# coganlab/cross_patient_speech_decoding

Hardware: AMD Instinct MI355X
Metric: ECoG trials/sec seq2seq-RNN training (higher is better)
Workload: dtype bf16x3; 1 GPU; configs[3] per-GPU shard: 8-patient MCCA-aligned input (d = 30), enc 2x bi-GRU H=512, dec 1x GRU, T=200 (T'=20), F=100, full-batch step of 2048 trials per GPU (8 patients x 2048 trials over 8 GPUs), dropout 0.3, teacher forcing 0.5, clip 0.5, AdamW; trials_per_gpu=2048, global_batch=2048, parallelism=dp1, collective=none (single process)

## Files before the change

### cross_patient_speech_decoding_amd/csrc/xps_common.h

```cpp
#pragma once
#include <hip/hip_runtime.h>
#include <stdint.h>
#include <stdio.h>
#include "../../include/xps.h"

typedef float f32x4 __attribute__((ext_vector_type(4)));
typedef float f32x16 __attribute__((ext_vector_type(16)));
typedef double f64x4 __attribute__((ext_vector_type(4)));

void xps_set_error(const char* fmt, ...);

#define XPS_CHECK_ARG(cond, msg)                                  \
    do {                                                          \
        if (!(cond)) {                                            \
            xps_set_error("%s: %s", __func__, msg);               \
            return XPS_E_INVALID;                                 \
        }                                                         \
    } while (0)

#define XPS_CHECK_LAUNCH()                                                        \
    do {                                                                          \
        hipError_t e_ = hipGetLastError();                                        \
        if (e_ != hipSuccess) {                                                   \
            xps_set_error("%s: launch failed: %s", __func__, hipGetErrorString(e_)); \
            return XPS_E_HIP;                                                     \
        }                                                                         \
    } while (0)

struct RowMap {
    long long gs, ld;
    int rpg;
    int fmt = 0;
    __host__ __device__ inline long long off(int i) const {
        return (long long)(i / rpg) * gs + (long long)(i % rpg) * ld;
    }
};

static inline RowMap to_rowmap(const xps_rowmap* r) {
    RowMap m;
    m.gs = r->gs;
    m.ld = r->ld;
    m.rpg = r->rpg < 1 ? 1 : r->rpg;
    m.fmt = r->fmt;
    return m;
}

static inline int cdiv(long long a, long long b) { return (int)((a + b - 1) / b); }

__device__ inline float sigmoidf_acc(float x) { return 1.0f / (1.0f + expf(-x)); }

__device__ inline void rng_pair(unsigned long long seed, long long pair, float& u0, float& u1) {
    unsigned long long z = seed + 0x9E3779B97F4A7C15ull * (unsigned long long)(pair + 1);
    z = (z ^ (z >> 30)) * 0xBF58476D1CE4E5B9ull;
    z = (z ^ (z >> 27)) * 0x94D049BB133111EBull;
    z ^= z >> 31;
    u0 = (float)((unsigned)(z >> 40)) * (1.0f / 16777216.0f);
    u1 = (float)((unsigned)(z >> 8) & 0xFFFFFFu) * (1.0f / 16777216.0f);
}
__device__ inline f32x4 split4_pack(const f32x4 v) {
    typedef __bf16 bf16x8_ __attribute__((ext_vector_type(8)));
    bf16x8_ o;
#pragma unroll
    for (int j = 0; j < 4; ++j) {
        const __bf16 h = (__bf16)v[j];
        o[j] = h;
        o[4 + j] = (__bf16)(v[j] - (float)h);
    }
    return __builtin_bit_cast(f32x4, o);
}
__device__ inline f32x4 dropout_keep4(unsigned long long seed, long long q, float p) {
    float u0, u1, u2, u3;
    rng_pair(seed, 2 * q, u0, u1);
    rng_pair(seed, 2 * q + 1, u2, u3);
    return (f32x4){u0 >= p ? 1.f : 0.f, u1 >= p ? 1.f : 0.f, u2 >= p ? 1.f : 0.f, u3 >= p ? 1.f : 0.f};
}

int xps_internal_gemm_mode();
```

### cross_patient_speech_decoding_amd/csrc/xps_gemm.hip

```cpp
#include <stdlib.h>
#include <string.h>
#include <atomic>
#include "xps_common.h"
#include "xps_gemm_tile.h"
#include "xps_gemm_big.h"
#include "xps_gemm_dma.h"
using namespace xps_tile;
#ifndef XPS_GEMM_DEFAULT_MODE
#define XPS_GEMM_DEFAULT_MODE 1
#endif
namespace {

#ifndef XPS_BF_MI1_WAVES
#define XPS_BF_MI1_WAVES XPS_GEMM_WAVES
#endif
template <bool AK, bool BK, int MI, bool EDGE = false, bool BF = false, bool PRE = false>
__global__ __launch_bounds__(256, (BF && MI == 1) ? XPS_BF_MI1_WAVES : XPS_GEMM_WAVES) void gemm_f32_kernel(
    const float* __restrict__ A, RowMap ra, const float* __restrict__ B, RowMap rb,
    const float* __restrict__ A2, const float* __restrict__ B2, int K2,
    float* __restrict__ C, RowMap rc, const float* __restrict__ bias,
    int M, int N, int K, int kchunk, long long slab_stride, int accumulate, int vecA, int vecB) {
    __shared__ __attribute__((aligned(16))) TileMem<BF, MI> mem;
    const int tiles_n = (N + BN - 1) / BN, tiles = tiles_n * ((M + 64 * MI - 1) / (64 * MI));
    const int lid = xcd_remap(blockIdx.x, gridDim.x);
    const int z = lid / tiles, t = lid % tiles;
    const int kbeg = z * kchunk;
    const int kend = min(K, kbeg + kchunk);
    const int m0 = (t / tiles_n) * (64 * MI), n0 = (t % tiles_n) * BN;
    f32x16 acc[MI][2];
    zero_acc<MI>(acc);
    float nocs = 0.f;
    f32x4 nocs4 = {0.f, 0.f, 0.f, 0.f};
    gemm_accumulate_any<AK, BK, MI, EDGE, BF, PRE>(acc, nocs, nocs4, false, A, ra, B, rb, M, N, K, m0, n0, kbeg, kend, vecA, vecB, mem);
    if (A2) gemm_accumulate_any<AK, BK, MI, EDGE, BF, PRE>(acc, nocs, nocs4, false, A2, ra, B2, rb, M, N, K2, m0, n0, 0, K2, vecA, vecB, mem);
    gemm_store<MI>(acc, C + (long long)z * slab_stride, rc, bias, M, N, m0, n0, accumulate);
}

constexpr int SM_MAXM = 16, SM_SLICES = 16, SM_KC = 1024;
template <bool AK, bool BK>
__global__ __launch_bounds__(1024) void gemm_small_kernel(
    const float* __restrict__ A, RowMap ra, const float* __restrict__ B, RowMap rb,
    const float* __restrict__ A2, const float* __restrict__ B2, int K2,
    float* __restrict__ C, RowMap rc, const float* __restrict__ bias, int M, int N, int K, int accumulate, int vecB) {
    __shared__ __attribute__((aligned(16))) float As[SM_MAXM][SM_KC];
    __shared__ float red[SM_SLICES][SM_MAXM][64];
    const int tid = threadIdx.x, l = tid & 63, w = tid >> 6;
    const int n = blockIdx.x * 64 + l;
    float acc[SM_MAXM];
#pragma unroll
    for (int m = 0; m < SM_MAXM; ++m) acc[m] = 0.f;
    for (int pass = 0; pass < 2; ++pass) {
        const float* __restrict__ Ap = pass ? A2 : A;
        const float* __restrict__ Bp = pass ? B2 : B;
        const int Kp = pass ? K2 : K;
        if (!Ap) break;
        const bool plain_b = rb.rpg >= Kp;
        for (int kc = 0; kc < Kp; kc += SM_KC) {
            const int kn = min(SM_KC, Kp - kc);
            __syncthreads();
            for (int e = tid; e < SM_MAXM * kn; e += 1024) {
                const int m = e / kn, k = e - m * kn;
                As[m][k] = m < M ? (AK ? Ap[ra.off(m) + kc + k] : Ap[ra.off(kc + k) + m]) : 0.f;
            }
            __syncthreads();
            const int kq = (((kn + SM_SLICES - 1) / SM_SLICES) + 3) & ~3;
            const int k0 = w * kq, k1 = min(kn, k0 + kq);
            if (n < N) {
                const long long boff = BK ? rb.off(n) + kc : (long long)n;
                int k = k0;
                for (; k + 3 < k1; k += 4) {
                    float b[4];
                    if (BK && vecB) {
                        const f32x4 v = *reinterpret_cast<const f32x4*>(Bp + boff + k);
                        b[0] = v.x; b[1] = v.y; b[2] = v.z; b[3] = v.w;
                    } else {
#pragma unroll
                        for (int j = 0; j < 4; ++j)
                            b[j] = BK ? Bp[boff + k + j]
                                      : Bp[(plain_b ? (long long)(kc + k + j) * rb.ld : rb.off(kc + k + j)) + boff];
                    }
#pragma unroll
                    for (int m = 0; m < SM_MAXM; ++m) {
                        const f32x4 a = *reinterpret_cast<const f32x4*>(&As[m][k]);
                        acc[m] += a.x * b[0]; acc[m] += a.y * b[1]; acc[m] += a.z * b[2]; acc[m] += a.w * b[3];
                    }
                }
                for (; k < k1; ++k) {
                    const float b = BK ? Bp[boff + k] : Bp[(plain_b ? (long long)(kc + k) * rb.ld : rb.off(kc + k)) + boff];
#pragma unroll
                    for (int m = 0; m < SM_MAXM; ++m) acc[m] += As[m][k] * b;
                }
            }
        }
    }
#pragma unroll
    for (int m = 0; m < SM_MAXM; ++m) red[w][m][l] = acc[m];
    __syncthreads();
    if (w < M && n < N) {
        float v = 0.f;
#pragma unroll
        for (int s = 0; s < SM_SLICES; ++s) v += red[s][w][l];
        if (bias) v += bias[n];
        float* c = C + rc.off(w) + n;
        if (accumulate) v += *c;
        *c = v;
    }
}

struct NtMulti {
    const float* B[4];
    const float* bias[4];
    float* C[4];
};
template <int MI, bool EDGE = false, bool BF = false, bool PRE = false>
__global__ __launch_bounds__(256, (BF && MI == 1) ? XPS_BF_MI1_WAVES : XPS_GEMM_WAVES) void gemm_nt_multi_kernel(
    const float* __restrict__ A, RowMap ra, NtMulti pm, RowMap rb, RowMap rc, int M, int N, int K, int nprob,
    int vecA, int vecB) {
    __shared__ __attribute__((aligned(16))) TileMem<BF, MI> mem;
    const int tiles_n = (N + BN - 1) / BN;
    const int lid = xcd_remap(blockIdx.x, gridDim.x);
    const int per_m = nprob * tiles_n, rem = lid % per_m;
    const int z = rem / tiles_n;
    const int m0 = (lid / per_m) * (64 * MI), n0 = (rem % tiles_n) * BN;
    f32x16 acc[MI][2];
    zero_acc<MI>(acc);
    float nocs = 0.f;
    f32x4 nocs4 = {0.f, 0.f, 0.f, 0.f};
    gemm_accumulate_any<true, true, MI, EDGE, BF, PRE>(acc, nocs, nocs4, false, A, ra, pm.B[z], rb, M, N, K, m0, n0, 0, K, vecA, vecB, mem);
    gemm_store<MI>(acc, pm.C[z], rc, pm.bias[z], M, N, m0, n0, 0);
}


template <int KT>
__global__ __launch_bounds__(512, 1) void proj_ws_kernel(const float* __restrict__ A, long long lda, NtMulti pm, long long ldb, long long ldc,
                                                         int M, int N, int K, int nprob, int preA, int preB) {
    constexpr int KP = 16 * KT;
#ifndef XPS_WS_PAD
#define XPS_WS_PAD 4
#endif
    constexpr int LDH = ((KP / 2 + 63) / 64) * 64 + XPS_WS_PAD;
    constexpr int NV = KP / 32;
    extern __shared__ __attribute__((aligned(16))) unsigned char ws_smem[];
    unsigned* lds = reinterpret_cast<unsigned*>(ws_smem);
    const int tid = threadIdx.x, lane = tid & 63, wave = tid >> 6;
    const int NC = nprob * N, S = (NC + 255) / 256;
    const int lid = xcd_remap(blockIdx.x, gridDim.x);
    const int slice = lid % S, rg = lid / S;
    const int nb = (gridDim.x - slice + S - 1) / S;
    const int c0 = slice * 256 + wave * 32;
    const bool active = c0 < NC;
    const int z = active ? c0 / N : 0, n0 = active ? c0 % N : 0;
    const int li = lane & 31, lk = lane >> 5;

    bf16x8 wh[KT], wl[KT];
    {
        const float* wrow = pm.B[z] + (long long)(n0 + li) * ldb;
#pragma unroll
        for (int kk = 0; kk < KT; ++kk) {
            const int k = 16 * kk + 8 * lk;
            f32x4 v0 = {0.f, 0.f, 0.f, 0.f}, v1 = v0;
            if (active && k < K) v0 = *reinterpret_cast<const f32x4*>(wrow + k);
            if (active && k + 4 < K) v1 = *reinterpret_cast<const f32x4*>(wrow + k + 4);
            bf16x4 h0, l0, h1, l1;
            stage_split(v0, preB != 0, h0, l0);
            stage_split(v1, preB != 0, h1, l1);
            wh[kk] = __builtin_shufflevector(h0, h1, 0, 1, 2, 3, 4, 5, 6, 7);
            wl[kk] = __builtin_shufflevector(l0, l1, 0, 1, 2, 3, 4, 5, 6, 7);
        }
    }
    float bv = 0.f;
    if (active && pm.bias[z]) bv = pm.bias[z][n0 + li];

    const int tiles = (M + 63) / 64;
    auto load_tile = [&](int t, f32x4 (&r)[NV]) {
#pragma unroll
        for (int j = 0; j < NV; ++j) {
            const int v = tid + 512 * j, row = t * 64 + v / (KP / 4), k = 4 * (v % (KP / 4));
            r[j] = (row < M && k < K) ? *reinterpret_cast<const f32x4*>(A + (long long)row * lda + k) : f32x4{0.f, 0.f, 0.f, 0.f};
        }
    };
    auto store_tile = [&](const f32x4 (&r)[NV], int buf) {
        unsigned* hi = lds + (size_t)buf * 2 * 64 * LDH;
        unsigned* lo = hi + 64 * LDH;
#pragma unroll
        for (int j = 0; j < NV; ++j) {
            const int v = tid + 512 * j, row = v / (KP / 4), kd = 2 * (v % (KP / 4));
            bf16x4 h, l;
            stage_split(r[j], preA != 0, h, l);
// ... 151 lines not shown
        for (int u = 0; u < 8; ++u) v[u] = p[(long long)(z + 4 * u) * stride];
#pragma unroll
        for (int u = 0; u < 8; ++u) s += v[u];
    }
    for (; z < splits; z += 4) s += p[(long long)z * stride];
    return s;
}

__device__ inline f32x4 slab_sum4(const float* __restrict__ p, long long stride, int splits, int w) {
    f32x4 s = {0.f, 0.f, 0.f, 0.f};
    int z = w;
    for (; z + 28 < splits; z += 32) {
        f32x4 v[8];
#pragma unroll
        for (int u = 0; u < 8; ++u) v[u] = *reinterpret_cast<const f32x4*>(p + (long long)(z + 4 * u) * stride);
#pragma unroll
        for (int u = 0; u < 8; ++u) s += v[u];
    }
    for (; z < splits; z += 4) s += *reinterpret_cast<const f32x4*>(p + (long long)z * stride);
    return s;
}

__global__ __launch_bounds__(256) void gemm_tn_grouped_reduce(TnGroup g, const float* __restrict__ ws) {
    __shared__ f32x4 part[4][RED_OUT];
    const int l = threadIdx.x & 63, w = threadIdx.x >> 6;
    const long long idx = ((long long)blockIdx.x * RED_OUT + l) * 4;
    const bool live = idx < g.total_out;
    int pi = 0;
    long long base = 0;
    if (live) {
#pragma unroll 1
        for (int i = 0; i < g.n; ++i) {
            const long long sz = tn_split_stride((long long)((g.p[i].M + BM - 1) / BM) * g.p[i].tiles_n, g.p[i].M, g.p[i].colsum != nullptr);
            if (idx < base + sz) { pi = i; break; }
            base += sz;
        }
    }
    const TnProb& P = g.p[pi];
    const long long tile_floats = (long long)((P.M + BM - 1) / BM) * P.tiles_n * TN_TILE;
    const long long split_stride = tn_split_stride(tile_floats / TN_TILE, P.M, P.colsum != nullptr);
    const long long e = idx - base;
    part[w][l] = live ? slab_sum4(ws + P.slab_off + e, split_stride, P.splits, w) : f32x4{0.f, 0.f, 0.f, 0.f};
    __syncthreads();
    if (w == 0 && live) {
        const f32x4 s4 = (part[0][l] + part[1][l]) + (part[2][l] + part[3][l]);
#pragma unroll
        for (int c = 0; c < 4; ++c) {
            float* dst = nullptr;
            bool is_cs = false;
            if (e < tile_floats) {
                const int tile = (int)(e / TN_TILE);
                int r, cc;
                slab_decode((int)(e % TN_TILE) + c, r, cc);
                const int row = (tile / P.tiles_n) * BM + r, col = (tile % P.tiles_n) * BN + cc;
                if (row < P.M && col < P.N)
                    dst = P.C + (P.rc.rpg >= P.M ? (long long)row * P.rc.ld : P.rc.off(row)) + col;
            } else {
                is_cs = true;
                if (e - tile_floats + c < P.M) dst = P.colsum + (e - tile_floats + c);
            }
            if (dst) {
                float s = s4[c];
                if ((P.accumulate & 1) || ((P.accumulate & 2) && is_cs)) s += *dst;
                *dst = s;
            }
        }
    }
}

__global__ __launch_bounds__(256) void gemm_tn_grouped_reduce_flat(TnGroup g, const float* __restrict__ ws) {
    const long long idx = ((long long)blockIdx.x * 256 + threadIdx.x) * 4;
    const bool live = idx < g.total_out;
    int pi = 0;
    long long base = 0;
    if (live) {
#pragma unroll 1
        for (int i = 0; i < g.n; ++i) {
            const long long sz = tn_split_stride((long long)((g.p[i].M + BM - 1) / BM) * g.p[i].tiles_n, g.p[i].M, g.p[i].colsum != nullptr);
            if (idx < base + sz) { pi = i; break; }
            base += sz;
        }
    }
    const TnProb& P = g.p[pi];
    const long long tile_floats = (long long)((P.M + BM - 1) / BM) * P.tiles_n * TN_TILE;
    const long long split_stride = tn_split_stride(tile_floats / TN_TILE, P.M, P.colsum != nullptr);
    const long long e = idx - base;
    if (live) {
        f32x4 s4 = {0.f, 0.f, 0.f, 0.f};
        const float* src = ws + P.slab_off + e;
        int z = 0;
        for (; z + 8 <= P.splits; z += 8) {
            f32x4 v[8];
#pragma unroll
            for (int u = 0; u < 8; ++u) v[u] = *reinterpret_cast<const f32x4*>(src + (long long)(z + u) * split_stride);
#pragma unroll
            for (int u = 0; u < 8; ++u) s4 += v[u];
        }
        {
            f32x4 v[8];
#pragma unroll
            for (int u = 0; u < 8; ++u)
                v[u] = z + u < P.splits ? *reinterpret_cast<const f32x4*>(src + (long long)(z + u) * split_stride) : f32x4{0.f, 0.f, 0.f, 0.f};
#pragma unroll
            for (int u = 0; u < 8; ++u) s4 += v[u];
        }
#pragma unroll
        for (int c = 0; c < 4; ++c) {
            float* dst = nullptr;
            bool is_cs = false;
            if (e < tile_floats) {
                const int tile = (int)(e / TN_TILE);
                int r, cc;
                slab_decode((int)(e % TN_TILE) + c, r, cc);
                const int row = (tile / P.tiles_n) * BM + r, col = (tile % P.tiles_n) * BN + cc;
                if (row < P.M && col < P.N)
                    dst = P.C + (P.rc.rpg >= P.M ? (long long)row * P.rc.ld : P.rc.off(row)) + col;
            } else {
                is_cs = true;
                if (e - tile_floats + c < P.M) dst = P.colsum + (e - tile_floats + c);
            }
            if (dst) {
                float s = s4[c];
                if ((P.accumulate & 1) || ((P.accumulate & 2) && is_cs)) s += *dst;
                *dst = s;
            }
        }
    }
}

extern __shared__ __attribute__((aligned(16))) unsigned char big_smem[];

template <bool AK, bool BK, bool DEEP, int FMT = -1>
__device__ inline void big_accumulate(f32x16 (&acc)[4][2], f32x4& csum, bool want_csum, const float* __restrict__ A, long long lda,
                                      const float* __restrict__ B, long long ldb, int m0, int n0, int kbeg, int kend,
                                      const bool preA = false, const bool preB = false) {
    if constexpr (DEEP) {
        xps_big::BigStage32& st = *reinterpret_cast<xps_big::BigStage32*>(big_smem);
        xps_big::BigLoader32<AK> la;
        xps_big::BigLoader32<BK> lb;
        la.init(A, lda, m0, kbeg, threadIdx.x);
        lb.init(B, ldb, n0, kbeg, threadIdx.x);
        xps_big::big_pipeline32<AK, BK>(acc, csum, want_csum, la, lb, (kend - kbeg) / 32, st, preA, preB);
    } else {
        xps_big::BigStage& st = *reinterpret_cast<xps_big::BigStage*>(big_smem);
        xps_big::BigLoader<AK> la;
        xps_big::BigLoader<BK> lb;
        la.init(A, lda, m0, kbeg, threadIdx.x);
        lb.init(B, ldb, n0, kbeg, threadIdx.x);
        if constexpr (FMT >= 0) xps_big::big_pipeline_t<AK, BK, (FMT & 1) != 0, (FMT & 2) != 0>(acc, csum, want_csum, la, lb, (kend - kbeg) / BKT, st);
        else xps_big::big_pipeline<AK, BK>(acc, csum, want_csum, la, lb, (kend - kbeg) / BKT, st, preA, preB);
    }
}

template <bool AK, bool BK, bool DEEP, int FMT = 0>
__global__ __launch_bounds__(512, 1) void gemm_big_kernel(const float* __restrict__ A, long long lda, const float* __restrict__ B,
                                                           long long ldb, const float* __restrict__ A2, const float* __restrict__ B2,
                                                           int K2, float* __restrict__ C, long long ldc,
                                                           const float* __restrict__ bias, int N, int K, int accumulate, int fmt) {
    const int tiles_n = FMT == 5 ? 1 : N / xps_big::TN;
    const int lid = xcd_remap(blockIdx.x, gridDim.x);
    const int m0 = (lid / tiles_n) * xps_big::TM, n0 = (lid % tiles_n) * xps_big::TN;
    f32x16 acc[4][2];
    xps_big::big_zero(acc);
    f32x4 nocs = {0.f, 0.f, 0.f, 0.f};
    if constexpr (FMT == 5) {
        const bool act = (int)((threadIdx.x >> 6) & 3) * 64 < N;
        xps_big::direct_dma_pipeline<!BK>(acc, A, lda, B, ldb, m0, 0, 0, K / 32, big_smem, act);
        if (A2) xps_big::direct_dma_pipeline<!BK>(acc, A2, lda, B2, ldb, m0, 0, 0, K2 / 32, big_smem, act);
        xps_big::big_store_c_masked(acc, C, ldc, bias, m0, N, accumulate);
        return;
    }
    if constexpr (FMT == 4) {
        xps_big::direct_dma_pipeline<!BK>(acc, A, lda, B, ldb, m0, n0, 0, K / 32, big_smem);
        if (A2) xps_big::direct_dma_pipeline<!BK>(acc, A2, lda, B2, ldb, m0, n0, 0, K2 / 32, big_smem);
    } else {
        big_accumulate<AK, BK, DEEP, DEEP ? -1 : FMT>(acc, nocs, false, A, lda, B, ldb, m0, n0, 0, K, !DEEP && (fmt & 1) != 0, !DEEP && (fmt & 2) != 0);
        if (A2) big_accumulate<AK, BK, DEEP, DEEP ? -1 : FMT>(acc, nocs, false, A2, lda, B2, ldb, m0, n0, 0, K2, !DEEP && (fmt & 1) != 0, !DEEP && (fmt & 2) != 0);
    }
    xps_big::big_store_c(acc, C, ldc, bias, m0, n0, accumulate);
}

template <bool DEEP, bool DMA = false>
__global__ __launch_bounds__(512, 1) void gemm_big_nt_multi_kernel(const float* __restrict__ A, long long lda, NtMulti pm, long long ldb,
                                                                    long long ldc, int N, int K, int nprob, int fmt) {
    const int tiles_n = N / xps_big::TN;
    const int lid = xcd_remap(blockIdx.x, gridDim.x);
    const int per_m = nprob * tiles_n, rem = lid % per_m;
    const int z = rem / tiles_n;
    const int m0 = (lid / per_m) * xps_big::TM, n0 = (rem % tiles_n) * xps_big::TN;
    f32x16 acc[4][2];
    xps_big::big_zero(acc);
    f32x4 nocs = {0.f, 0.f, 0.f, 0.f};
    if constexpr (DMA) xps_big::direct_dma_pipeline<false>(acc, A, lda, pm.B[z], ldb, m0, n0, 0, K / 32, big_smem);
    else big_accumulate<true, true, DEEP>(acc, nocs, false, A, lda, pm.B[z], ldb, m0, n0, 0, K, !DEEP && (fmt & 1) != 0, !DEEP && (fmt & 2) != 0);
    xps_big::big_store_c(acc, pm.C[z], ldc, pm.bias[z], m0, n0, 0);
}

template <bool DEEP>
__global__ __launch_bounds__(512, 1) void gemm_big_tn_kernel(TnGroup g, float* __restrict__ ws) {
    const int lid = xcd_remap(blockIdx.x, gridDim.x);
    int pi = -1;
#pragma unroll 1
    for (int i = 0; i < g.n; ++i)
        if (g.p[i].big && lid >= g.p[i].block_start) pi = i;
    const TnProb& P = g.p[pi];
    const int local = lid - P.block_start;
    const int tiles_n = P.N / xps_big::TN, ntiles = (P.M / xps_big::TM) * tiles_n;
    const int tile = local % ntiles, z = local / ntiles;
    const int tm = tile / tiles_n, tn = tile % tiles_n;
    const int kbeg = z * P.kchunk, kend = min(P.K, kbeg + P.kchunk);
    const long long ntiles128 = (long long)(P.M / BM) * P.tiles_n;
    const long long split_stride = tn_split_stride(ntiles128, P.M, P.colsum != nullptr);
    float* slab = ws + P.slab_off + (long long)z * split_stride;
    const bool want_cs = P.colsum && tn == 0;
    f32x16 acc[4][2];
    xps_big::big_zero(acc);
    if (!DEEP && P.big == 2) {
        f32x16 cacc;
#pragma unroll
        for (int r = 0; r < 16; ++r) cacc[r] = 0.f;
        const int per = (8 + tiles_n - 1) / tiles_n;
        const int cs_lo = min(8, tn * per), cs_hi = min(8, cs_lo + per);
        const bool cs_here = P.colsum && cs_lo < cs_hi;
        if (cs_here) xps_big::tn_dma_pipeline<true>(acc, cacc, P.A, P.ra.ld, P.B, P.rb.ld, tm * xps_big::TM, tn * xps_big::TN, kbeg, (kend - kbeg) / BKT, big_smem, cs_lo, cs_hi);
        else xps_big::tn_dma_pipeline<false>(acc, cacc, P.A, P.ra.ld, P.B, P.rb.ld, tm * xps_big::TM, tn * xps_big::TN, kbeg, (kend - kbeg) / BKT, big_smem);
        float* subd[4];
#pragma unroll
        for (int s = 0; s < 4; ++s)
            subd[s] = slab + ((long long)(2 * tm + (s >> 1)) * P.tiles_n + 2 * tn + (s & 1)) * TN_TILE;
        xps_big::big_slab_store(acc, subd);
        if (cs_here) xps_big::dma_colsum_store(cacc, slab + ntiles128 * TN_TILE + tm * xps_big::TM, cs_lo, cs_hi);
        return;
    }
    f32x4 csum = {0.f, 0.f, 0.f, 0.f};
    big_accumulate<false, false, DEEP>(acc, csum, want_cs, P.A, P.ra.ld, P.B, P.rb.ld, tm * xps_big::TM, tn * xps_big::TN, kbeg, kend,
                                       !DEEP && (P.vecA & 2) != 0, !DEEP && (P.vecB & 2) != 0);
    float* sub[4];
#pragma unroll
    for (int s = 0; s < 4; ++s)
        sub[s] = slab + ((long long)(2 * tm + (s >> 1)) * P.tiles_n + 2 * tn + (s & 1)) * TN_TILE;
    xps_big::big_slab_store(acc, sub);
    if (want_cs) {
        float* red = reinterpret_cast<float*>(big_smem);
        const int tid = threadIdx.x;
        *reinterpret_cast<f32x4*>(&red[(tid >> 6) * 256 + (tid & 63) * 4]) = csum;
        __syncthreads();
        if (tid < 256) {
            float v = 0.f;
#pragma unroll
            for (int w = 0; w < 8; ++w) v += red[w * 256 + tid];
            slab[ntiles128 * TN_TILE + tm * xps_big::TM + tid] = v;
        }
    }
}

__global__ __launch_bounds__(256) void splitk_reduce_kernel(const float* __restrict__ slabs, int splits, long long slab_stride,
                                                            float* __restrict__ C, RowMap rc, int M, int N, int accumulate) {
    __shared__ float part[4][RED_OUT];
    const int l = threadIdx.x & 63, w = threadIdx.x >> 6;
    const long long idx = (long long)blockIdx.x * RED_OUT + l;
    const bool live = idx < (long long)M * N;
    part[w][l] = live ? slab_sum(slabs + idx, slab_stride, splits, w) : 0.f;
    __syncthreads();
    if (w == 0 && live) {
        float s = (part[0][l] + part[1][l]) + (part[2][l] + part[3][l]);
        float* p = C + rc.off((int)(idx / N)) + (int)(idx % N);
        if (accumulate) s += *p;
        *p = s;
    }
}

inline bool aligned16(const void* p) { return (reinterpret_cast<uintptr_t>(p) & 15) == 0; }
inline bool map_vec_ok(const float* p, const RowMap& r) {
    return aligned16(p) && (r.ld % 4 == 0) && (r.gs % 4 == 0);
}
inline int split4_flag(const float* p, const RowMap& r, long long extent) {
    if (r.fmt == 0) return 0;
    if (r.fmt != 1 || !map_vec_ok(p, r) || extent % 4 != 0) return -1;
    return 2;
}

int tn_splits(int M, int N, int K) {
    long long tiles = (long long)cdiv(M, BM) * cdiv(N, BN);
    int want = (int)((768 + tiles - 1) / tiles);
    int maxs = cdiv(K, 256);
    int s = want < maxs ? want : maxs;
    if (s < 1) s = 1;
    if (s > 256) s = 256;
    return s;
}

}

namespace {
std::atomic<int>& gemm_mode() {
    static std::atomic<int> mode([] {
        const char* e = getenv("XPS_GEMM_PRECISION");
        if (e && (!strcmp(e, "fp32") || !strcmp(e, "f32") || !strcmp(e, "0"))) return 0;
        if (e && (!strcmp(e, "bf16x3") || !strcmp(e, "1"))) return 1;
        return XPS_GEMM_DEFAULT_MODE;
    }());
    return mode;
}
inline bool bf_mode() { return gemm_mode().load(std::memory_order_relaxed) == 1; }

inline bool use_small_tiles(int M, int N, int K = 0) {
    static const int thr = [] {
        const char* e = getenv("XPS_GEMM_SMALL_TILE_BLOCKS");
        int v = e ? atoi(e) : -1;
        return v >= 0 ? v : 2048;
    }();
    const long long n128 = (long long)cdiv(M, 128) * cdiv(N, BN);
    static const bool longk = [] { const char* e = getenv("XPS_GEMM_LONGK_128"); return !(e && e[0] == '0'); }();
    if (longk && K >= 1024 && n128 >= 512) return false;
    return M > 64 && n128 < thr;
}

std::atomic<int>& big_switch() {
    static std::atomic<int> on([] { const char* e = getenv("XPS_GEMM_BIG"); return (e && e[0] == '0') ? 0 : 1; }());
    return on;
}
inline bool big_enabled() { return big_switch().load(std::memory_order_relaxed) != 0 && bf_mode(); }
inline bool dma_enabled() { const char* e = getenv("XPS_GEMM_DMA"); return !(e && e[0] == '0'); }
inline bool proj_ws_enabled() { const char* e = getenv("XPS_PROJ_WS"); return !(e && e[0] == '0'); }
inline bool big_plain(const float* p, const RowMap& r, int rows) { return aligned16(p) && r.ld % 4 == 0 && r.rpg >= rows; }
constexpr int BIG_LDS = (int)sizeof(xps_big::BigStage), BIG_LDS32 = (int)sizeof(xps_big::BigStage32);
constexpr int BIG_TN_LDS = BIG_LDS > xps_big::DMA_LDS ? BIG_LDS : xps_big::DMA_LDS;
template <typename Kern>
inline bool big_prepare(Kern kern, int bytes) {
    return hipFuncSetAttribute(reinterpret_cast<const void*>(kern), hipFuncAttributeMaxDynamicSharedMemorySize, bytes) == hipSuccess;
}
inline bool big_deep_allowed() {
    static const bool on = [] { const char* e = getenv("XPS_GEMM_BIG_DEEP"); return e && e[0] == '1'; }();
    return on;
}
inline int big_min_tiles() {
    static const int v = [] { const char* e = getenv("XPS_GEMM_BIG_MIN_TILES"); int x = e ? atoi(e) : 0; return x > 0 ? x : 192; }();
    return v;
}

inline int device_cus() {
    static const int cus = [] {
        int dev = 0, n = 0;
        if (hipGetDevice(&dev) == hipSuccess && hipDeviceGetAttribute(&n, hipDeviceAttributeMultiprocessorCount, dev) == hipSuccess && n > 0) return n;
        return 256;
    }();
    return cus;
}
inline int big_split_rows(int M, int tiles_per_row_tile) {
    static const bool on = [] { const char* e = getenv("XPS_GEMM_BIG_TAIL"); return !(e && e[0] == '0'); }();
    const int cus = device_cus();
    const long long mt = M / xps_big::TM, total = mt * tiles_per_row_tile;
    const long long rounds = total / cus, rem = total % cus;
    if (!on || rounds < 1 || rem == 0 || rem * 4 > (long long)cus * 3) return M;
    const long long mb = (rounds * cus) / tiles_per_row_tile;
    if (mb < 1 || mb >= mt) return M;
    return (int)(mb * xps_big::TM);
}

template <bool AK, bool BK>
int launch_gemm(const float* A, const RowMap& ra, const float* B, const RowMap& rb, const float* A2, const float* B2, int K2,
                float* C, const RowMap& rc, const float* bias, int M, int N, int K, int accumulate, hipStream_t st) {
    const int kchunk = ((K + BKT - 1) / BKT) * BKT + BKT;
    int vecA = (int)(map_vec_ok(A, ra) && (!A2 || map_vec_ok(A2, ra)));
    int vecB = (int)(map_vec_ok(B, rb) && (!B2 || map_vec_ok(B2, rb)));
    int fA = split4_flag(A, ra, AK ? K : M), fB = split4_flag(B, rb, BK ? K : N);
    if (A2 && fA > 0) fA = split4_flag(A2, ra, AK ? K2 : M);
    if (B2 && fB > 0) fB = split4_flag(B2, rb, BK ? K2 : N);
    if (fA < 0 || fB < 0 || ((fA | fB) && (!bf_mode() || M <= SM_MAXM))) return -2;
    vecA |= fA; vecB |= fB;
    const int fmt = (fA ? 1 : 0) | (fB ? 2 : 0);
    if (M <= SM_MAXM) {
        hipLaunchKernelGGL((gemm_small_kernel<AK, BK>), dim3(cdiv(N, 64)), dim3(1024), 0, st, A, ra, B, rb, A2, B2, K2, C, rc,
                           bias, M, N, K, accumulate, vecB);
        return hipGetLastError() == hipSuccess ? 0 : -1;
    }
    if constexpr (AK && !BK) {
        if (big_enabled() && dma_enabled() && fmt == 3 && N < xps_big::TN && N % 4 == 0 && rb.ld >= xps_big::TN && M % xps_big::TM == 0 &&
            M / xps_big::TM >= 96 && K % 32 == 0 && K2 % 32 == 0 && K + K2 >= 512 && big_plain(A, ra, M) && big_plain(B, rb, K) &&
            (!A2 || (big_plain(A2, ra, M) && big_plain(B2, rb, K2))) && rc.rpg >= M) {
            constexpr int lds = xps_big::direct_dma_lds<true>();
            static const bool ready5 = big_prepare(gemm_big_kernel<true, false, false, 5>, lds);
            if (ready5) {
                hipLaunchKernelGGL((gemm_big_kernel<true, false, false, 5>), dim3(M / xps_big::TM), dim3(xps_big::NTHR), lds, st,
                                   A, ra.ld, B, rb.ld, A2, B2, K2, C, rc.ld, bias, N, K, accumulate, fmt);
                return hipGetLastError() == hipSuccess ? 0 : -1;
            }
        }
    }
    if (big_enabled() && M % xps_big::TM == 0 && N % xps_big::TN == 0 && K % BKT == 0 && K2 % BKT == 0 && K >= 64 &&
        (long long)(M / xps_big::TM) * (N / xps_big::TN) >= big_min_tiles() &&
        big_plain(A, ra, AK ? M : K) && big_plain(B, rb, BK ? N : K) && (!A2 || (big_plain(A2, ra, AK ? M : K2) && big_plain(B2, rb, BK ? N : K2))) &&
        rc.rpg >= M) {
        static const bool ready = big_prepare(gemm_big_kernel<AK, BK, false, 0>, BIG_LDS) && big_prepare(gemm_big_kernel<AK, BK, false, 1>, BIG_LDS) &&
                                  big_prepare(gemm_big_kernel<AK, BK, false, 2>, BIG_LDS) && big_prepare(gemm_big_kernel<AK, BK, false, 3>, BIG_LDS) &&
                                  big_prepare(gemm_big_kernel<AK, BK, true>, BIG_LDS32);
        if (ready) {
            const int Mfull = M;
            M = big_split_rows(M, N / xps_big::TN);
            const dim3 bgrid((M / xps_big::TM) * (N / xps_big::TN));
            const int Mtail = Mfull - M;
            auto run_tail = [&]() -> int {
                if (Mtail <= 0) return 0;
                const float* At = AK ? A + (long long)M * ra.ld : A + M;
                const float* A2t = A2 ? (AK ? A2 + (long long)M * ra.ld : A2 + M) : nullptr;
                return launch_gemm<AK, BK>(At, ra, B, rb, A2t, B2, K2, C + (long long)M * rc.ld, rc, bias, Mtail, N, K, accumulate, st);
            };
            bool dma_done = false;
            if constexpr (AK) {
                if (fmt == 3 && K % 32 == 0 && K2 % 32 == 0 && dma_enabled()) {
                    constexpr int lds = xps_big::direct_dma_lds<!BK>();
                    static const bool ready4 = big_prepare(gemm_big_kernel<AK, BK, false, 4>, lds);
                    if (ready4) {
                        hipLaunchKernelGGL((gemm_big_kernel<AK, BK, false, 4>), bgrid, dim3(xps_big::NTHR), lds, st,
                                           A, ra.ld, B, rb.ld, A2, B2, K2, C, rc.ld, bias, N, K, accumulate, fmt);
                        dma_done = true;
                    }
                }
            }
            if (dma_done) {
            } else if (big_deep_allowed() && K % 32 == 0 && K2 % 32 == 0 && fmt == 0)
                hipLaunchKernelGGL((gemm_big_kernel<AK, BK, true>), bgrid, dim3(xps_big::NTHR), BIG_LDS32, st,
                                   A, ra.ld, B, rb.ld, A2, B2, K2, C, rc.ld, bias, N, K, accumulate, fmt);
            else if (fmt == 0)
                hipLaunchKernelGGL((gemm_big_kernel<AK, BK, false, 0>), bgrid, dim3(xps_big::NTHR), BIG_LDS, st,
                                   A, ra.ld, B, rb.ld, A2, B2, K2, C, rc.ld, bias, N, K, accumulate, fmt);
            else if (fmt == 1)
                hipLaunchKernelGGL((gemm_big_kernel<AK, BK, false, 1>), bgrid, dim3(xps_big::NTHR), BIG_LDS, st,
                                   A, ra.ld, B, rb.ld, A2, B2, K2, C, rc.ld, bias, N, K, accumulate, fmt);
            else if (fmt == 2)
                hipLaunchKernelGGL((gemm_big_kernel<AK, BK, false, 2>), bgrid, dim3(xps_big::NTHR), BIG_LDS, st,
                                   A, ra.ld, B, rb.ld, A2, B2, K2, C, rc.ld, bias, N, K, accumulate, fmt);
            else
                hipLaunchKernelGGL((gemm_big_kernel<AK, BK, false, 3>), bgrid, dim3(xps_big::NTHR), BIG_LDS, st,
                                   A, ra.ld, B, rb.ld, A2, B2, K2, C, rc.ld, bias, N, K, accumulate, fmt);
            if (hipGetLastError() != hipSuccess) return -1;
            return run_tail();
        }
    }
#define XPS_LAUNCH_GEMM(MI_, EDGE_, BF_)                                                                              \
    do {                                                                                                              \
        if (BF_ && fmt)                                                                                               \
            hipLaunchKernelGGL((gemm_f32_kernel<AK, BK, MI_, EDGE_, BF_, BF_>), grid, dim3(256), 0, st, A, ra, B, rb, A2, B2, K2, C, rc, \
                               bias, M, N, K, kchunk, 0LL, accumulate, vecA, vecB);                                   \
        else                                                                                                          \
            hipLaunchKernelGGL((gemm_f32_kernel<AK, BK, MI_, EDGE_, BF_>), grid, dim3(256), 0, st, A, ra, B, rb, A2, B2, K2, C, rc, \
                               bias, M, N, K, kchunk, 0LL, accumulate, vecA, vecB);                                   \
    } while (0)
    const bool bf = bf_mode();
    if (use_small_tiles(M, N, K + K2)) {
        dim3 grid(cdiv(N, BN) * cdiv(M, 64));
        const bool edge = (M % 64) || (N % BN);
        if (bf) { if (edge) XPS_LAUNCH_GEMM(1, true, true); else XPS_LAUNCH_GEMM(1, false, true); }
        else { if (edge) XPS_LAUNCH_GEMM(1, true, false); else XPS_LAUNCH_GEMM(1, false, false); }
    } else {
        dim3 grid(cdiv(N, BN) * cdiv(M, 128));
        const bool edge = (M % 128) || (N % BN);
        if (bf) { if (edge) XPS_LAUNCH_GEMM(2, true, true); else XPS_LAUNCH_GEMM(2, false, true); }
        else { if (edge) XPS_LAUNCH_GEMM(2, true, false); else XPS_LAUNCH_GEMM(2, false, false); }
    }
#undef XPS_LAUNCH_GEMM
    return hipGetLastError() == hipSuccess ? 0 : -1;
}
}

extern "C" int xps_gemm_nt_f32(const float* A, const xps_rowmap* ra_, const float* B, const xps_rowmap* rb_,
                               float* C, const xps_rowmap* rc_, const float* bias,
                               int M, int N, int K, int accumulate, void* stream) {
    XPS_CHECK_ARG(A && B && C && ra_ && rb_ && rc_, "null argument");
    XPS_CHECK_ARG(M >= 0 && N >= 0 && K >= 0, "negative size");
    if (M == 0 || N == 0) return XPS_OK;
    RowMap ra = to_rowmap(ra_), rb = to_rowmap(rb_), rc = to_rowmap(rc_);
    const int lrc = launch_gemm<true, true>(A, ra, B, rb, nullptr, nullptr, 0, C, rc, bias, M, N, K, accumulate, (hipStream_t)stream);
    if (lrc == -2) {
        xps_set_error("xps_gemm_nt_f32: XPS_FMT_SPLIT4 operand needs bf16x3 mode, M > 16, 16-byte aligned rows and a contiguous extent that is a multiple of 4");
        return XPS_E_INVALID;
    }
    if (lrc) {
        xps_set_error("xps_gemm_nt_f32: launch failed: %s", hipGetErrorString(hipGetLastError()));
        return XPS_E_HIP;
    }
    return XPS_OK;
}

extern "C" int xps_gemm_nn_f32(const float* A, const xps_rowmap* ra_, const float* B, const xps_rowmap* rb_,
                               float* C, const xps_rowmap* rc_,
                               int M, int N, int K, int accumulate, void* stream) {
    XPS_CHECK_ARG(A && B && C && ra_ && rb_ && rc_, "null argument");
    XPS_CHECK_ARG(M >= 0 && N >= 0 && K >= 0, "negative size");
    if (M == 0 || N == 0) return XPS_OK;
    RowMap ra = to_rowmap(ra_), rb = to_rowmap(rb_), rc = to_rowmap(rc_);
    const int lrc = launch_gemm<true, false>(A, ra, B, rb, nullptr, nullptr, 0, C, rc, nullptr, M, N, K, accumulate, (hipStream_t)stream);
    if (lrc == -2) {
        xps_set_error("xps_gemm_nn_f32: XPS_FMT_SPLIT4 operand needs bf16x3 mode, M > 16, 16-byte aligned rows and a contiguous extent that is a multiple of 4");
        return XPS_E_INVALID;
    }
    if (lrc) {
        xps_set_error("xps_gemm_nn_f32: launch failed: %s", hipGetErrorString(hipGetLastError()));
        return XPS_E_HIP;
    }
    return XPS_OK;
}

extern "C" int xps_gemm_nt_multi_f32(const float* A, const xps_rowmap* ra_, const float* const* B, const xps_rowmap* rb_,
                                     float* const* C, const xps_rowmap* rc_, const float* const* bias, int nprob,
                                     int M, int N, int K, void* stream) {
    XPS_CHECK_ARG(A && B && C && ra_ && rb_ && rc_, "null argument");
    XPS_CHECK_ARG(nprob >= 1 && nprob <= 4, "1..4 problems");
    XPS_CHECK_ARG(M >= 0 && N >= 0 && K >= 0, "negative size");
    if (M == 0 || N == 0) return XPS_OK;
    RowMap ra = to_rowmap(ra_), rb = to_rowmap(rb_), rc = to_rowmap(rc_);
    NtMulti pm;
    bool vb = true;
    for (int i = 0; i < 4; ++i) {
        const int j = i < nprob ? i : 0;
        XPS_CHECK_ARG(B[j] && C[j], "null problem pointer");
        pm.B[i] = B[j]; pm.C[i] = C[j]; pm.bias[i] = bias ? bias[j] : nullptr;
        vb = vb && map_vec_ok(B[j], rb);
    }
    int vecA = (int)map_vec_ok(A, ra), vecB = (int)vb;
    int fA = split4_flag(A, ra, K), fB = 0;
    for (int i = 0; i < nprob && fB >= 0; ++i) fB = split4_flag(B[i], rb, K);
    if (fA < 0 || fB < 0 || ((fA | fB) && !bf_mode())) {
        xps_set_error("xps_gemm_nt_multi_f32: XPS_FMT_SPLIT4 operand needs bf16x3 mode, 16-byte aligned rows and K %% 4 == 0");
        return XPS_E_INVALID;
    }
    vecA |= fA; vecB |= fB;
    const int fmt = (fA ? 1 : 0) | (fB ? 2 : 0);
    if (bf_mode() && proj_ws_enabled() && K >= 32 && K <= 256 && K % 4 == 0 && N % 32 == 0 && (long long)nprob * N >= 256 && M >= 4096 &&
        vecA && vb && ra.rpg >= M && rb.rpg >= N && rc.rpg >= M) {
        const int KT = 2 * ((K + 31) / 32);
        static const int cus = [] {
            int dev = 0, n = 0;
            if (hipGetDevice(&dev) == hipSuccess && hipDeviceGetAttribute(&n, hipDeviceAttributeMultiprocessorCount, dev) == hipSuccess && n > 0) return n;
            return 256;
        }();
        const int S = cdiv((long long)nprob * N, 256), tiles = cdiv(M, 64);
        int grid = cus < tiles * S ? cus : tiles * S;
        grid = (grid / S) * S;
        if (grid >= S) {
#define XPS_LAUNCH_WS(KT_)                                                                                                            \
    do {                                                                                                                              \
        static const bool ok_ = big_prepare(proj_ws_kernel<KT_>, proj_ws_lds(KT_));                                                    \
        if (!ok_) { xps_set_error("xps_gemm_nt_multi_f32: cannot reserve %d bytes of LDS", proj_ws_lds(KT_)); return XPS_E_HIP; }       \
        hipLaunchKernelGGL(proj_ws_kernel<KT_>, dim3(grid), dim3(512), proj_ws_lds(KT_), (hipStream_t)stream, A, ra.ld, pm, rb.ld, rc.ld, \
                           M, N, K, nprob, fA ? 1 : 0, fB ? 1 : 0);                                                                      \
    } while (0)
            switch (KT) {
                case 2: XPS_LAUNCH_WS(2); break;
                case 4: XPS_LAUNCH_WS(4); break;
                case 6: XPS_LAUNCH_WS(6); break;
                case 8: XPS_LAUNCH_WS(8); break;
                case 10: XPS_LAUNCH_WS(10); break;
                case 12: XPS_LAUNCH_WS(12); break;
                case 14: XPS_LAUNCH_WS(14); break;
                default: XPS_LAUNCH_WS(16); break;
            }
#undef XPS_LAUNCH_WS
            XPS_CHECK_LAUNCH();
            return XPS_OK;
        }
    }
    if (big_enabled() && M % xps_big::TM == 0 && N % xps_big::TN == 0 && K % BKT == 0 && K >= 64 && vb &&
        (long long)(M / xps_big::TM) * (N / xps_big::TN) * nprob >= big_min_tiles() &&
        big_plain(A, ra, M) && rb.rpg >= N && rc.rpg >= M) {
        static const bool ready = big_prepare(gemm_big_nt_multi_kernel<false>, BIG_LDS) && big_prepare(gemm_big_nt_multi_kernel<true>, BIG_LDS32);
        if (ready) {
            const int Mfull = M;
            M = big_split_rows(M, (N / xps_big::TN) * nprob);
            const dim3 bgrid((M / xps_big::TM) * (N / xps_big::TN) * nprob);
            static const bool ready_dma = big_prepare(gemm_big_nt_multi_kernel<false, true>, xps_big::direct_dma_lds<false>());
            if (fmt == 3 && K % 32 == 0 && dma_enabled() && ready_dma)
                hipLaunchKernelGGL((gemm_big_nt_multi_kernel<false, true>), bgrid, dim3(xps_big::NTHR), xps_big::direct_dma_lds<false>(),
                                   (hipStream_t)stream, A, ra.ld, pm, rb.ld, rc.ld, N, K, nprob, fmt);
            else if (big_deep_allowed() && K % 32 == 0 && fmt == 0)
                hipLaunchKernelGGL(gemm_big_nt_multi_kernel<true>, bgrid, dim3(xps_big::NTHR), BIG_LDS32, (hipStream_t)stream, A, ra.ld, pm,
                                   rb.ld, rc.ld, N, K, nprob, fmt);
            else
                hipLaunchKernelGGL(gemm_big_nt_multi_kernel<false>, bgrid, dim3(xps_big::NTHR), BIG_LDS,
                               (hipStream_t)stream, A, ra.ld, pm, rb.ld, rc.ld, N, K, nprob, fmt);
            XPS_CHECK_LAUNCH();
            if (Mfull > M) {
                float* Ct[4];
                for (int i = 0; i < nprob; ++i) Ct[i] = C[i] + (long long)M * rc.ld;
                return xps_gemm_nt_multi_f32(A + (long long)M * ra.ld, ra_, B, rb_, Ct, rc_, bias, nprob, Mfull - M, N, K, stream);
            }
            return XPS_OK;
        }
    }
#define XPS_LAUNCH_NTM(MI_, EDGE_, BF_)                                                                                  \
    do {                                                                                                                 \
        if (BF_ && fmt)                                                                                                  \
            hipLaunchKernelGGL((gemm_nt_multi_kernel<MI_, EDGE_, BF_, BF_>), dim3(cdiv(N, BN) * cdiv(M, 64 * MI_) * nprob), dim3(256), 0, \
                               (hipStream_t)stream, A, ra, pm, rb, rc, M, N, K, nprob, vecA, vecB);                        \
        else                                                                                                             \
            hipLaunchKernelGGL((gemm_nt_multi_kernel<MI_, EDGE_, BF_>), dim3(cdiv(N, BN) * cdiv(M, 64 * MI_) * nprob), dim3(256), 0,    \
                               (hipStream_t)stream, A, ra, pm, rb, rc, M, N, K, nprob, vecA, vecB);                        \
    } while (0)
    const bool bf = bf_mode();
    if (use_small_tiles(M, N * nprob, K)) {
        const bool edge = (M % 64) || (N % BN);
        if (bf) { if (edge) XPS_LAUNCH_NTM(1, true, true); else XPS_LAUNCH_NTM(1, false, true); }
        else { if (edge) XPS_LAUNCH_NTM(1, true, false); else XPS_LAUNCH_NTM(1, false, false); }
    } else {
        const bool edge = (M % 128) || (N % BN);
        if (bf) { if (edge) XPS_LAUNCH_NTM(2, true, true); else XPS_LAUNCH_NTM(2, false, true); }
        else { if (edge) XPS_LAUNCH_NTM(2, true, false); else XPS_LAUNCH_NTM(2, false, false); }
    }
#undef XPS_LAUNCH_NTM
    XPS_CHECK_LAUNCH();
    return XPS_OK;
}

extern "C" int xps_gemm_nn2_f32(const float* A1, const float* B1, int K1, const float* A2, const float* B2, int K2,
                                const xps_rowmap* ra_, const xps_rowmap* rb_, float* C, const xps_rowmap* rc_,
                                int M, int N, int accumulate, void* stream) {
    XPS_CHECK_ARG(A1 && B1 && A2 && B2 && C && ra_ && rb_ && rc_, "null argument");
    XPS_CHECK_ARG(M >= 0 && N >= 0 && K1 >= 0 && K2 >= 0, "negative size");
    if (M == 0 || N == 0) return XPS_OK;
    RowMap ra = to_rowmap(ra_), rb = to_rowmap(rb_), rc = to_rowmap(rc_);
    const int lrc = launch_gemm<true, false>(A1, ra, B1, rb, A2, B2, K2, C, rc, nullptr, M, N, K1, accumulate, (hipStream_t)stream);
    if (lrc == -2) {
        xps_set_error("xps_gemm_nn2_f32: XPS_FMT_SPLIT4 operand needs bf16x3 mode, M > 16, 16-byte aligned rows and a contiguous extent that is a multiple of 4");
        return XPS_E_INVALID;
    }
    if (lrc) {
        xps_set_error("xps_gemm_nn2_f32: launch failed: %s", hipGetErrorString(hipGetLastError()));
        return XPS_E_HIP;
    }
    return XPS_OK;
}

extern "C" size_t xps_gemm_tn_f32_workspace(int M, int N, int K) {
    if (M <= 0 || N <= 0 || K <= 0) return 16;
    int s = tn_splits(M, N, K);
    return (size_t)s * (size_t)M * (size_t)N * sizeof(float) + 16;
}

extern "C" int xps_gemm_tn_f32(const float* A, const xps_rowmap* ra_, const float* B, const xps_rowmap* rb_,
                               float* C, const xps_rowmap* rc_,
                               int M, int N, int K, int accumulate,
                               void* workspace, size_t workspace_bytes, void* stream) {
    XPS_CHECK_ARG(A && B && C && ra_ && rb_ && rc_, "null argument");
    XPS_CHECK_ARG(M >= 0 && N >= 0 && K >= 0, "negative size");
    if (M == 0 || N == 0) return XPS_OK;
    RowMap ra = to_rowmap(ra_), rb = to_rowmap(rb_), rc = to_rowmap(rc_);
    XPS_CHECK_ARG(ra.fmt == 0 && rb.fmt == 0, "XPS_FMT_SPLIT4 operands: use xps_gemm_tn_grouped_f32");
    const int splits = (K > 0) ? tn_splits(M, N, K) : 1;
    if (workspace_bytes < xps_gemm_tn_f32_workspace(M, N, K) || !workspace) {
        xps_set_error("xps_gemm_tn_f32: workspace too small (%zu < %zu)", workspace_bytes,
                      xps_gemm_tn_f32_workspace(M, N, K));
        return XPS_E_WORKSPACE;
    }
    XPS_CHECK_ARG(aligned16(workspace), "workspace must be 16-byte aligned");
    int kchunk = ((cdiv(K > 0 ? K : 1, splits) + BKT - 1) / BKT) * BKT;
    float* slabs = reinterpret_cast<float*>(workspace);
    RowMap rs;
    rs.gs = 0; rs.ld = N; rs.rpg = 1 << 30;
    const long long slab_stride = (long long)M * N;
    dim3 grid(cdiv(N, BN) * cdiv(M, BM) * splits);
    if (bf_mode())
        hipLaunchKernelGGL((gemm_f32_kernel<false, false, 2, true, true>), grid, dim3(256), 0, (hipStream_t)stream,
                           A, ra, B, rb, (const float*)nullptr, (const float*)nullptr, 0, slabs, rs, (const float*)nullptr,
                           M, N, K, kchunk, slab_stride, 0, (int)map_vec_ok(A, ra), (int)map_vec_ok(B, rb));
    else
        hipLaunchKernelGGL((gemm_f32_kernel<false, false, 2>), grid, dim3(256), 0, (hipStream_t)stream,
                           A, ra, B, rb, (const float*)nullptr, (const float*)nullptr, 0, slabs, rs, (const float*)nullptr,
                           M, N, K, kchunk, slab_stride, 0, (int)map_vec_ok(A, ra), (int)map_vec_ok(B, rb));
    XPS_CHECK_LAUNCH();
    long long total = (long long)M * N;
    hipLaunchKernelGGL(splitk_reduce_kernel, dim3(cdiv(total, RED_OUT)), dim3(256), 0, (hipStream_t)stream,
                       slabs, splits, slab_stride, C, rc, M, N, accumulate);
    XPS_CHECK_LAUNCH();
    return XPS_OK;
}

namespace {
int build_group(const xps_tn_problem* probs, int n, TnGroup& g, size_t& ws_floats, int big_choice = -1) {
    if (n < 1 || n > TN_MAXP) return -1;
    static const int target_blocks = [] {
        const char* e = getenv("XPS_TN_BLOCKS");
        int v = e ? atoi(e) : 0;
        return v > 0 ? v : 512;
    }();
    const bool big_on = big_choice < 0 ? big_enabled() : big_choice != 0;
    bool isbig[TN_MAXP];
    long long tiles_total = 0, tiles_big_total = 0;
    for (int i = 0; i < n; ++i) {
        const xps_tn_problem& q = probs[i];
        if (!q.A || !q.B || !q.C || q.M < 1 || q.N < 1 || q.K < 0) return -1;
        const RowMap ra = to_rowmap(&q.ra), rb = to_rowmap(&q.rb);
        isbig[i] = big_on && q.M % xps_big::TM == 0 && q.N % xps_big::TN == 0 && q.K % BKT == 0 && q.K >= 4096 &&
                   big_plain(q.A, ra, q.K) && big_plain(q.B, rb, q.K);
        if (isbig[i]) tiles_big_total += (long long)(q.M / xps_big::TM) * (q.N / xps_big::TN);
        else tiles_total += (long long)cdiv(q.M, BM) * cdiv(q.N, BN);
    }
    int sp_big = 1;
    if (tiles_big_total > 0) {
        const int r1 = (int)(256 / tiles_big_total), r2 = (int)(512 / tiles_big_total);
        sp_big = (r1 >= 1 && r1 * tiles_big_total >= 230) ? r1 : (r2 >= 1 ? r2 : 1);
    }
    g.n = n;
    int blocks = 0, blocks_big = 0;
    long long off = 0, out = 0;
    for (int i = 0; i < n; ++i) {
        const xps_tn_problem& q = probs[i];
        TnProb& P = g.p[i];
        P.A = q.A; P.B = q.B; P.C = q.C; P.colsum = q.colsum_a;
        P.ra = to_rowmap(&q.ra); P.rb = to_rowmap(&q.rb); P.rc = to_rowmap(&q.rc);
        P.M = q.M; P.N = q.N; P.K = q.K; P.accumulate = q.accumulate;
        const int tiles = cdiv(q.M, BM) * cdiv(q.N, BN);
        const long long split_stride = tn_split_stride(tiles, q.M, q.colsum_a != nullptr);
        int sp;
        if (isbig[i]) {
            sp = sp_big;
            const int maxs = q.K / 512;
            if (sp > maxs) sp = maxs;
        } else {
            int want = (int)((target_blocks * (long long)tiles / (tiles_total > 0 ? tiles_total : 1) + tiles - 1) / tiles);
            int maxs = cdiv(q.K > 0 ? q.K : 1, 64);
            sp = want < maxs ? want : maxs;
        }
        if (sp < 1) sp = 1;
        if (sp > 256) sp = 256;
        P.splits = sp;
        const int kq = (isbig[i] && q.K % 32 == 0) ? 32 : BKT;
        P.kchunk = ((cdiv(q.K > 0 ? q.K : 1, sp) + kq - 1) / kq) * kq;
        P.tiles_n = cdiv(q.N, BN);
        const int fA = split4_flag(q.A, P.ra, q.M), fB = split4_flag(q.B, P.rb, q.N);
        if (fA < 0 || fB < 0 || ((fA | fB) && !bf_mode())) return -2;
        P.vecA = (int)map_vec_ok(q.A, P.ra) | fA;
        P.vecB = (int)map_vec_ok(q.B, P.rb) | fB;
        P.slab_off = off;
        P.big = isbig[i] ? ((fA && fB && dma_enabled()) ? 2 : 1) : 0;
        if (isbig[i]) {
            P.block_start = blocks_big;
            blocks_big += (q.M / xps_big::TM) * (q.N / xps_big::TN) * sp;
        } else {
            P.block_start = blocks;
            blocks += tiles * sp;
        }
        off += (long long)sp * split_stride;
        out += split_stride;
    }
    g.total_blocks_big = blocks_big;
    g.total_blocks = blocks;
    g.total_out = out;
    ws_floats = (size_t)off;
    g.uniform = 0;
    g.tiles_all = 0;
    bool same_k = n > 1;
    for (int i = 1; i < n; ++i) same_k = same_k && probs[i].K == probs[0].K;
    static const bool allow = [] { const char* e = getenv("XPS_TN_UNIFORM"); return e && e[0] == '1'; }();
    if (same_k && allow && probs[0].K > 0 && blocks_big == 0) {
        int sp = (int)((target_blocks + tiles_total - 1) / tiles_total);
        const int maxs = cdiv(probs[0].K, 64);
        if (sp > maxs) sp = maxs;
        if (sp < 1) sp = 1;
        if (sp > 256) sp = 256;
        const int kchunk = ((cdiv(probs[0].K, sp) + BKT - 1) / BKT) * BKT;
        blocks = 0; off = 0;
        int tstart = 0;
        for (int i = 0; i < n; ++i) {
            TnProb& P = g.p[i];
            const int tiles = cdiv(P.M, BM) * cdiv(P.N, BN);
            P.splits = sp; P.kchunk = kchunk;
            P.slab_off = off;
            P.block_start = blocks;
            g.tile_start[i] = tstart;
            tstart += tiles;
            blocks += tiles * sp;
            off += (long long)sp * tn_split_stride(tiles, P.M, P.colsum != nullptr);
        }
        for (int i = n; i < TN_MAXP; ++i) g.tile_start[i] = 1 << 30;
        g.tiles_all = tstart;
        g.total_blocks = blocks;
        ws_floats = (size_t)off;
        g.uniform = 1;
    }
    return 0;
}
}

extern "C" size_t xps_gemm_tn_grouped_f32_workspace(const xps_tn_problem* probs, int n) {
    TnGroup g;
    size_t fl0 = 0, fl1 = 0;
    if (!probs || build_group(probs, n, g, fl0, 0) || build_group(probs, n, g, fl1, 1)) return 0;
    return (fl0 > fl1 ? fl0 : fl1) * sizeof(float) + 16;
}

extern "C" int xps_gemm_tn_grouped_f32(const xps_tn_problem* probs, int n, void* workspace, size_t workspace_bytes,
                                       void* stream) {
    XPS_CHECK_ARG(probs, "null argument");
    TnGroup g;
    size_t fl = 0;
    if (build_group(probs, n, g, fl)) {
        xps_set_error("xps_gemm_tn_grouped_f32: invalid problem list (1..%d problems, non-null pointers, M,N >= 1; XPS_FMT_SPLIT4 "
                      "operands: bf16x3 mode, 16-byte aligned rows, M / N multiples of 4)", TN_MAXP);
        return XPS_E_INVALID;
    }
    if (!workspace || workspace_bytes < fl * sizeof(float) + 16 || !aligned16(workspace)) {
        xps_set_error("xps_gemm_tn_grouped_f32: workspace too small or misaligned");
        return XPS_E_WORKSPACE;
    }
    bool edge = false;
    for (int i = 0; i < n; ++i) edge = edge || (!g.p[i].big && ((probs[i].M % BM) || (probs[i].N % BN)));
    const bool bf = bf_mode();
    bool anypre = false;
    for (int i = 0; i < n; ++i) anypre = anypre || (!g.p[i].big && ((g.p[i].vecA | g.p[i].vecB) & 2));
    if (g.total_blocks_big > 0) {
        static const bool ready = big_prepare(gemm_big_tn_kernel<false>, BIG_TN_LDS) && big_prepare(gemm_big_tn_kernel<true>, BIG_LDS32);
        if (!ready) {
            xps_set_error("xps_gemm_tn_grouped_f32: cannot reserve %d bytes of LDS", BIG_LDS32 > BIG_TN_LDS ? BIG_LDS32 : BIG_TN_LDS);
            return XPS_E_HIP;
        }
        static const bool deep_tn = [] { const char* e = getenv("XPS_GEMM_BIG_DEEP_TN"); return e && e[0] == '1'; }();
        bool deep = big_deep_allowed() && deep_tn;
        for (int i = 0; i < n; ++i) deep = deep && (!g.p[i].big || (g.p[i].kchunk % 32 == 0 && g.p[i].K % 32 == 0 && !((g.p[i].vecA | g.p[i].vecB) & 2)));
        if (deep)
            hipLaunchKernelGGL(gemm_big_tn_kernel<true>, dim3(g.total_blocks_big), dim3(xps_big::NTHR), BIG_LDS32, (hipStream_t)stream, g,
                               (float*)workspace);
// ... 56 lines not shown
```

### cross_patient_speech_decoding_amd/csrc/xps_gemm_big.h

```cpp
#pragma once
#include "xps_gemm_tile.h"

namespace xps_big {
using namespace xps_tile;

constexpr int TM = 256, TN = 256, NTHR = 512;

constexpr int BIG_NS = 2;
struct BigStage {
    BfTile<256> a[BIG_NS];
    BfTile<256> b[BIG_NS];
};

template <bool KC>
struct BigLoader {
    const float* p[2];
    long long kstep;
    __device__ inline void init(const float* __restrict__ P, long long ld, int x0, int k0, int tid) {
        if (KC) {
#pragma unroll
            for (int r = 0; r < 2; ++r) p[r] = P + (long long)(x0 + (tid >> 2) + 128 * r) * ld + k0 + (tid & 3) * 4;
            kstep = BKT;
        } else {
#pragma unroll
// ... 155 lines not shown
template <bool KC>
__device__ inline void big_stage32(const f32x4 (&v)[4], Image32& S, int tid, const bool pre) {
#pragma unroll
    for (int r = 0; r < 4; ++r) {
        bf16x4 h, l;
        stage_split(v[r], pre, h, l);
        if (KC) {
            const int row = (tid >> 3) + 64 * r, kc = tid & 7, c4 = kc & 3;
            const int col = (((c4 >> 1) ^ ((row >> 3) & 1)) << 3) + ((c4 & 1) << 2);
            if (kc < 4) {
                *reinterpret_cast<bf16x4*>(&S.kc.hi0[row][col]) = h;
                *reinterpret_cast<bf16x4*>(&S.kc.lo0[row][col]) = l;
            } else {
                *reinterpret_cast<bf16x4*>(&S.kc.hi1[row][col]) = h;
                *reinterpret_cast<bf16x4*>(&S.kc.lo1[row][col]) = l;
            }
        } else {
            const int k = (tid >> 6) + 8 * r, x4 = (tid & 63) * 4;
            *reinterpret_cast<bf16x4*>(&S.kx.thi[k][x4]) = h;
            *reinterpret_cast<bf16x4*>(&S.kx.tlo[k][x4]) = l;
        }
    }
}

template <bool KC>
__device__ inline void big_frag32(const Image32& S, int t, int x0, int lane, bf16x8& fh, bf16x8& fl) {
    if constexpr (KC) {
        const int row = x0 + (lane & 31), col = (((lane >> 5) ^ ((row >> 3) & 1)) << 3);
        if (t == 0) {
            fh = *reinterpret_cast<const bf16x8*>(&S.kc.hi0[row][col]);
            fl = *reinterpret_cast<const bf16x8*>(&S.kc.lo0[row][col]);
        } else {
            fh = *reinterpret_cast<const bf16x8*>(&S.kc.hi1[row][col]);
            fl = *reinterpret_cast<const bf16x8*>(&S.kc.lo1[row][col]);
        }
    } else {
        typedef __attribute__((address_space(3))) bf16x4 lds_bf16x4;
        const int g = lane >> 4, i = lane & 15, q = i >> 2, pp = i & 3;
        const int k0 = 16 * t + 8 * (g >> 1) + q, c0 = x0 + (g & 1) * 16 + 4 * pp;
        const bf16x4 h0 = __builtin_amdgcn_ds_read_tr16_b64_v4bf16((lds_bf16x4*)(&S.kx.thi[k0][c0]));
        const bf16x4 h1 = __builtin_amdgcn_ds_read_tr16_b64_v4bf16((lds_bf16x4*)(&S.kx.thi[k0 + 4][c0]));
        const bf16x4 l0 = __builtin_amdgcn_ds_read_tr16_b64_v4bf16((lds_bf16x4*)(&S.kx.tlo[k0][c0]));
        const bf16x4 l1 = __builtin_amdgcn_ds_read_tr16_b64_v4bf16((lds_bf16x4*)(&S.kx.tlo[k0 + 4][c0]));
        fh = __builtin_shufflevector(h0, h1, 0, 1, 2, 3, 4, 5, 6, 7);
        fl = __builtin_shufflevector(l0, l1, 0, 1, 2, 3, 4, 5, 6, 7);
    }
}

template <bool AK, bool BK>
__device__ inline void big_mma32(f32x16 (&acc)[4][2], const BigStage32& S, int buf) {
    const int lane = threadIdx.x & 63, wave = threadIdx.x >> 6;
    const int wm = (wave >> 2) * 128, wn = (wave & 3) * 64;
#pragma unroll
    for (int t = 0; t < 2; ++t) {
        bf16x8 bh[2], bl[2];
#pragma unroll
        for (int j = 0; j < 2; ++j) big_frag32<BK>(S.b[buf], t, wn + j * 32, lane, bh[j], bl[j]);
#pragma unroll
        for (int i = 0; i < 4; ++i) {
            bf16x8 ah, al;
            big_frag32<AK>(S.a[buf], t, wm + i * 32, lane, ah, al);
#pragma unroll
            for (int j = 0; j < 2; ++j) {
                acc[i][j] = __builtin_amdgcn_mfma_f32_32x32x16_bf16(al, bh[j], acc[i][j], 0, 0, 0);
                acc[i][j] = __builtin_amdgcn_mfma_f32_32x32x16_bf16(ah, bl[j], acc[i][j], 0, 0, 0);
                acc[i][j] = __builtin_amdgcn_mfma_f32_32x32x16_bf16(ah, bh[j], acc[i][j], 0, 0, 0);
            }
        }
    }
}

template <bool AK, bool BK>
__device__ inline void big_pipeline32(f32x16 (&acc)[4][2], f32x4& csum, const bool want_csum, const BigLoader32<AK>& la,
                                      const BigLoader32<BK>& lb, const int nks, BigStage32& S, const bool preA, const bool preB) {
    const int tid = threadIdx.x;
    if (nks <= 0) return;
    f32x4 va[4], vb[4];
    la.load(va, 0); lb.load(vb, 0);
    big_stage32<AK>(va, S.a[0], tid, preA);
    big_stage32<BK>(vb, S.b[0], tid, preB);
    if (!AK && want_csum) csum += (stage_values(va[0], preA) + stage_values(va[1], preA)) + (stage_values(va[2], preA) + stage_values(va[3], preA));
    __syncthreads();
    int ks = 0;
    for (; ks + 1 < nks; ++ks) {
        const int buf = ks & 1;
        la.load(va, ks + 1); lb.load(vb, ks + 1);
        __builtin_amdgcn_sched_barrier(0);
        big_mma32<AK, BK>(acc, S, buf);
        big_stage32<AK>(va, S.a[buf ^ 1], tid, preA);
        big_stage32<BK>(vb, S.b[buf ^ 1], tid, preB);
        if (!AK && want_csum) csum += (stage_values(va[0], preA) + stage_values(va[1], preA)) + (stage_values(va[2], preA) + stage_values(va[3], preA));
        __syncthreads();
    }
    big_mma32<AK, BK>(acc, S, ks & 1);
    __syncthreads();
}

__device__ inline void big_zero(f32x16 (&acc)[4][2]) {
#pragma unroll
    for (int i = 0; i < 4; ++i)
#pragma unroll
        for (int j = 0; j < 2; ++j)
#pragma unroll
            for (int r = 0; r < 16; ++r) acc[i][j][r] = 0.f;
}

__device__ inline void big_store_c(const f32x16 (&acc)[4][2], float* __restrict__ C, long long ldc, const float* __restrict__ bias,
                                   int m0, int n0, int accumulate) {
    const int lane = threadIdx.x & 63, wave = threadIdx.x >> 6;
    const int wm = (wave >> 2) * 128, wn = (wave & 3) * 64;
    const int li = lane & 31, lk = lane >> 5;
    float* cbase = C + (long long)(m0 + wm + 4 * lk) * ldc + n0 + wn + li;
    float bv[2] = {0.f, 0.f};
    if (bias) { bv[0] = bias[n0 + wn + li]; bv[1] = bias[n0 + wn + 32 + li]; }
#pragma unroll
    for (int i = 0; i < 4; ++i)
#pragma unroll
        for (int r = 0; r < 16; ++r) {
            float* crow = cbase + (long long)(i * 32 + (r & 3) + 8 * (r >> 2)) * ldc;
#pragma unroll
            for (int j = 0; j < 2; ++j) {
                float v = acc[i][j][r] + bv[j];
                if (accumulate) v += crow[j * 32];
                __builtin_nontemporal_store(v, &crow[j * 32]);
            }
        }
}

__device__ inline void big_store_c_masked(const f32x16 (&acc)[4][2], float* __restrict__ C, long long ldc, const float* __restrict__ bias,
                                          int m0, int nvalid, int accumulate) {
    const int lane = threadIdx.x & 63, wave = threadIdx.x >> 6;
    const int wm = (wave >> 2) * 128, wn = (wave & 3) * 64;
    const int li = lane & 31, lk = lane >> 5;
    if (wn >= nvalid) return;
    float* cbase = C + (long long)(m0 + wm + 4 * lk) * ldc + wn + li;
    const bool ok[2] = {wn + li < nvalid, wn + 32 + li < nvalid};
    float bv[2] = {0.f, 0.f};
    if (bias) { bv[0] = ok[0] ? bias[wn + li] : 0.f; bv[1] = ok[1] ? bias[wn + 32 + li] : 0.f; }
#pragma unroll
    for (int i = 0; i < 4; ++i)
#pragma unroll
        for (int r = 0; r < 16; ++r) {
            float* crow = cbase + (long long)(i * 32 + (r & 3) + 8 * (r >> 2)) * ldc;
#pragma unroll
            for (int j = 0; j < 2; ++j) {
                if (!ok[j]) continue;
                float v = acc[i][j][r] + bv[j];
                if (accumulate) v += crow[j * 32];
                __builtin_nontemporal_store(v, &crow[j * 32]);
            }
        }
}

__device__ inline void big_slab_store(const f32x16 (&acc)[4][2], float* const (&sub)[4]) {
    const int lane = threadIdx.x & 63, wave = threadIdx.x >> 6;
    float* base = sub[(wave >> 2) * 2 + ((wave & 3) >> 1)] + lane * 4;
#pragma unroll
    for (int i = 0; i < 4; ++i)
#pragma unroll
        for (int j = 0; j < 2; ++j)
#pragma unroll
            for (int q = 0; q < 4; ++q) {
                const f32x4 v = {acc[i][j][4 * q], acc[i][j][4 * q + 1], acc[i][j][4 * q + 2], acc[i][j][4 * q + 3]};
                const int wave_o = (i >> 1) * 2 + (wave & 1);
                __builtin_nontemporal_store(v, reinterpret_cast<f32x4*>(base + wave_o * 4096 + (((i & 1) * 2 + j) * 4 + q) * 256));
            }
}

}
```

### cross_patient_speech_decoding_amd/csrc/xps_gemm_tile.h

```cpp
#pragma once
#include "xps_common.h"

namespace xps_tile {

#ifndef XPS_BKT
#define XPS_BKT 16
#endif
#ifndef XPS_GEMM_WAVES
#define XPS_GEMM_WAVES 1
#endif
constexpr int BM = 128, BN = 128, BKT = XPS_BKT, LDT = 132;

#ifdef XPS_GSTAMP
static __device__ unsigned long long g_gstamp[8192 * 4];
#define GSTAMP(var)                                                                  \
    __builtin_amdgcn_sched_barrier(0);                                               \
    asm volatile("s_memtime %0\n\ts_waitcnt lgkmcnt(0)" : "=s"(var)::"memory");      \
    __builtin_amdgcn_sched_barrier(0);
#else
#define GSTAMP(var)
#endif

constexpr int KL = BKT / 4;

// ... 349 lines not shown
    f32x4 ra0[LA::NV], rb0[LB::NV], ra1[LA::NV], rb1[LB::NV];
    if (nkt > 0) {
        if (MODE) { la.template load_fast<MODE == 2>(ra0, kbeg); lb.template load_fast<MODE == 2>(rb0, kbeg); }
        else { la.load(ra0, A, ra, m0, M, kbeg, kend, tid, vecA); lb.load(rb0, B, rb, n0, N, kbeg, kend, tid, vecB); }
        if (nkt > 1) {
            if (MODE) { la.template load_fast<MODE == 2>(ra1, kbeg + BKT); lb.template load_fast<MODE == 2>(rb1, kbeg + BKT); }
            else { la.load(ra1, A, ra, m0, M, kbeg + BKT, kend, tid, vecA); lb.load(rb1, B, rb, n0, N, kbeg + BKT, kend, tid, vecB); }
        }
        bf_store<AK, WM>(ra0, S.a[0], tid, preA);
        bf_store<BK, 128>(rb0, S.b[0], tid, preB);
        if (want_csum) bf_colsum<AK, WM>(ra0, csum, preA);
    }
    __syncthreads();
#ifdef XPS_GSTAMP
    unsigned long long g0 = 0, g1 = 0, g2 = 0, g3 = 0, g4 = 0, s_ld = 0, s_mm = 0, s_st = 0, s_bar = 0;
#endif
    for (int kt = 0; kt < nkt; ++kt) {
        const int buf = kt & 1;
        GSTAMP(g0)
        if (kt + 2 < nkt) {
            if (MODE) { la.template load_fast<MODE == 2>(ra0, kbeg + (kt + 2) * BKT); lb.template load_fast<MODE == 2>(rb0, kbeg + (kt + 2) * BKT); }
            else { la.load(ra0, A, ra, m0, M, kbeg + (kt + 2) * BKT, kend, tid, vecA); lb.load(rb0, B, rb, n0, N, kbeg + (kt + 2) * BKT, kend, tid, vecB); }
        }
        GSTAMP(g1)
        {
            bf16x8 ah[MI], al[MI], bh[2], bl[2];
#pragma unroll
            for (int i = 0; i < MI; ++i) bf_frag<AK, 64 * MI>(S.a[buf], wm + i * 32, lane, ah[i], al[i]);
#pragma unroll
            for (int j = 0; j < 2; ++j) bf_frag<BK, 128>(S.b[buf], wn + j * 32, lane, bh[j], bl[j]);
#pragma unroll
            for (int i = 0; i < MI; ++i)
#pragma unroll
                for (int j = 0; j < 2; ++j) {
                    acc[i][j] = __builtin_amdgcn_mfma_f32_32x32x16_bf16(al[i], bh[j], acc[i][j], 0, 0, 0);
                    acc[i][j] = __builtin_amdgcn_mfma_f32_32x32x16_bf16(ah[i], bl[j], acc[i][j], 0, 0, 0);
                    acc[i][j] = __builtin_amdgcn_mfma_f32_32x32x16_bf16(ah[i], bh[j], acc[i][j], 0, 0, 0);
                }
        }
        GSTAMP(g2)
        if (kt + 1 < nkt) {
            bf_store<AK, WM>(ra1, S.a[buf ^ 1], tid, preA);
            bf_store<BK, 128>(rb1, S.b[buf ^ 1], tid, preB);
            if (want_csum) bf_colsum<AK, WM>(ra1, csum, preA);
#pragma unroll
            for (int r = 0; r < LA::NV; ++r) ra1[r] = ra0[r];
#pragma unroll
            for (int r = 0; r < LB::NV; ++r) rb1[r] = rb0[r];
        }
        GSTAMP(g3)
        __syncthreads();
#ifdef XPS_GSTAMP
        GSTAMP(g4)
        s_ld += g1 - g0; s_mm += g2 - g1; s_st += g3 - g2; s_bar += g4 - g3;
#endif
    }
#ifdef XPS_GSTAMP
    if (lane == 0) {
        const int wid = (((blockIdx.y * gridDim.x + blockIdx.x) * 4 + wave)) & 8191;
        g_gstamp[wid * 4 + 0] = s_ld; g_gstamp[wid * 4 + 1] = s_mm; g_gstamp[wid * 4 + 2] = s_st; g_gstamp[wid * 4 + 3] = s_bar;
    }
#endif
}

template <bool AK, bool BK, int MI, bool EDGE = false, bool ANYPRE = false>
__device__ inline void gemm_accumulate_bf(f32x16 (&acc)[MI][2], f32x4& csum, const bool want_csum,
                                          const float* __restrict__ A, const RowMap& ra, const float* __restrict__ B, const RowMap& rb,
                                          int M, int N, int K, int m0, int n0, int kbeg, int kend, int vecA, int vecB, BfStage<MI>& S) {
    TileLoader<AK, 64 * MI, true> la;
    TileLoader<BK, 128, true> lb;
    la.init(A, ra, m0, M, K, threadIdx.x, vecA);
    lb.init(B, rb, n0, N, K, threadIdx.x, vecB);
    const int kfull = kbeg + ((kend - kbeg) / BKT) * BKT;
    const bool both_fast = la.fast && lb.fast && kfull > kbeg;
    const bool both_full = la.full && lb.full;
    if (both_fast && both_full) {
        gemm_pipeline_bf<AK, BK, MI, 1, ANYPRE>(acc, csum, want_csum, la, lb, A, ra, B, rb, M, N, m0, n0, kbeg, kfull, vecA, vecB, S);
        if (kfull < kend)
            gemm_pipeline_bf<AK, BK, MI, 0, ANYPRE>(acc, csum, want_csum, la, lb, A, ra, B, rb, M, N, m0, n0, kfull, kend, vecA, vecB, S);
    } else if (EDGE && both_fast && !both_full) {
        gemm_pipeline_bf<AK, BK, MI, 2, ANYPRE>(acc, csum, want_csum, la, lb, A, ra, B, rb, M, N, m0, n0, kbeg, kfull, vecA, vecB, S);
        if (kfull < kend)
            gemm_pipeline_bf<AK, BK, MI, 0, ANYPRE>(acc, csum, want_csum, la, lb, A, ra, B, rb, M, N, m0, n0, kfull, kend, vecA, vecB, S);
    } else {
        gemm_pipeline_bf<AK, BK, MI, 0, ANYPRE>(acc, csum, want_csum, la, lb, A, ra, B, rb, M, N, m0, n0, kbeg, kend, vecA, vecB, S);
    }
}

template <bool BF, int MI = 2> struct TileMem;
template <int MI> struct TileMem<false, MI> {
    float As[2][BKT][LDT];
    float Bs[2][BKT][LDT];
};
template <int MI> struct TileMem<true, MI> {
    BfStage<MI> st;
};
template <bool AK, bool BK, int MI, bool EDGE, bool BF, bool ANYPRE = false>
__device__ inline void gemm_accumulate_any(f32x16 (&acc)[MI][2], float& csum, f32x4& csum4, const bool want_csum,
                                           const float* __restrict__ A, const RowMap& ra, const float* __restrict__ B, const RowMap& rb,
                                           int M, int N, int K, int m0, int n0, int kbeg, int kend, int vecA, int vecB,
                                           TileMem<BF, MI>& mem) {
    if constexpr (BF) gemm_accumulate_bf<AK, BK, MI, EDGE, ANYPRE>(acc, csum4, want_csum, A, ra, B, rb, M, N, K, m0, n0, kbeg, kend, vecA, vecB, mem.st);
    else gemm_accumulate<AK, BK, MI, EDGE>(acc, csum, want_csum, A, ra, B, rb, M, N, K, m0, n0, kbeg, kend, vecA, vecB, mem.As, mem.Bs);
}

template <int MI>
__device__ inline void gemm_store(const f32x16 (&acc)[MI][2], float* __restrict__ C, const RowMap& rc,
                                  const float* __restrict__ bias, int M, int N, int m0, int n0, int accumulate) {
    const int lane = threadIdx.x & 63, wave = threadIdx.x >> 6;
    const int wm = (wave >> 1) * (32 * MI), wn = (wave & 1) * 64;
    const int li = lane & 31, lk = lane >> 5;
    if (rc.rpg >= M && m0 + 64 * MI <= M && n0 + 128 <= N) {
        float* cbase = C + (long long)(m0 + wm + 4 * lk) * rc.ld + n0 + wn + li;
        float bv[2] = {0.f, 0.f};
        if (bias) { bv[0] = bias[n0 + wn + li]; bv[1] = bias[n0 + wn + 32 + li]; }
#pragma unroll
        for (int i = 0; i < MI; ++i)
#pragma unroll
            for (int r = 0; r < 16; ++r) {
                float* crow = cbase + (long long)(i * 32 + (r & 3) + 8 * (r >> 2)) * rc.ld;
#pragma unroll
                for (int j = 0; j < 2; ++j) {
                    float v = acc[i][j][r] + bv[j];
                    if (accumulate) v += crow[j * 32];
                    __builtin_nontemporal_store(v, &crow[j * 32]);
                }
            }
        return;
    }
    const bool plain = rc.rpg >= M;
    const int c0 = n0 + wn + li, c1 = c0 + 32;
    float bv[2] = {0.f, 0.f};
    if (bias) { bv[0] = c0 < N ? bias[c0] : 0.f; bv[1] = c1 < N ? bias[c1] : 0.f; }
#pragma unroll
    for (int i = 0; i < MI; ++i) {
#pragma unroll
        for (int r = 0; r < 16; ++r) {
            const int row = m0 + wm + i * 32 + (r & 3) + 8 * (r >> 2) + 4 * lk;
            if (row >= M) continue;
            float* crow = C + (plain ? (long long)row * rc.ld : rc.off(row));
#pragma unroll
            for (int j = 0; j < 2; ++j) {
                const int col = j ? c1 : c0;
                if (col < N) {
                    float v = acc[i][j][r] + bv[j];
                    if (accumulate) v += crow[col];
                    __builtin_nontemporal_store(v, &crow[col]);
                }
            }
        }
    }
}

template <int MI>
__device__ inline void zero_acc(f32x16 (&acc)[MI][2]) {
#pragma unroll
    for (int i = 0; i < MI; ++i)
#pragma unroll
        for (int j = 0; j < 2; ++j)
#pragma unroll
            for (int r = 0; r < 16; ++r) acc[i][j][r] = 0.f;
}


}
```

### cross_patient_speech_decoding_amd/nn_models/functional.py

```python
import ctypes as C
import os
from typing import NamedTuple

import torch

from .._dev import need_gpu as _need_gpu, ptr as _ptr, ptr_array as _ptr_array, stream as _stream, workspace as _ws
from .._lib import TnProblem, call, lib, rowmap

_f32 = torch.float32

GEMM_PRECISIONS = {'fp32': 0, 'bf16x3': 1}


def set_gemm_precision(name):
    if name not in GEMM_PRECISIONS:
        raise ValueError(f"gemm precision must be one of {sorted(GEMM_PRECISIONS)}")
    call('xps_set_gemm_precision', GEMM_PRECISIONS[name])


def get_gemm_precision():
    mode = lib().xps_get_gemm_precision()
    return {v: k for k, v in GEMM_PRECISIONS.items()}[mode]


# ... 296 lines not shown
    nbytes = _gru_ws_bytes('xps_gru_seq_fwd_f32_workspace', T, B, H, ndir)
    ws = _ws(nbytes, dev)
    _gru_status_register(dev)
    call('xps_gru_seq_fwd_images_f32', _ptr(gi), _ptr_array(w_hh), _ptr_array(b_hh), None, _ptr(y_ext), _ptr(saved), T, B, H, ndir,
         _ptr(y_split), _ptr(yd_split), float(drop[0]) if (drop and want_dropped) else 0.0, int(drop[1]) if (drop and want_dropped) else 0,
         _ptr(ws), nbytes, _stream())
    return y_ext, saved, y_split, yd_split


def gru_forward_training_form(gi, w_hh, b_hh, T, B, H, ndir):
    if fwd_ysplit_wanted(T, B, H, ndir):
        return _gru_forward_images(gi, w_hh, b_hh, T, B, H, ndir, True, False, None)[:2]
    return _gru_forward(gi, w_hh, b_hh, None, T, B, H, ndir, True)


def _gru_backward(dy, dhn, y_ext, saved, w_hh, T, B, H, ndir, need_dh0, drop=None, split4=False, form=None):
    dev = y_ext.device
    _check_form(form if form is not None else getattr(saved, 'launch_form', None), B, H)
    if dy is not None and not dy.is_contiguous():
        dy = dy.contiguous()
    if dhn is not None and not dhn.is_contiguous():
        dhn = dhn.contiguous()
    if dy is None and dhn is None:
        dhn = torch.zeros(ndir, B, H, dtype=_f32, device=dev)
    if len(w_hh) > 1:
        w_t = [torch.empty(H, 3 * H, dtype=_f32, device=dev) for _ in w_hh]
        call('xps_transpose_batched_f32', _ptr_array(w_hh), _ptr_array(w_t), len(w_hh), 3 * H, H, _stream())
    else:
        w_t = [transpose(w, 3 * H, H) for w in w_hh]
    dgi = torch.empty(ndir, T, B, 3 * H, dtype=_f32, device=dev)
    dghn = torch.empty(ndir, T, B, H, dtype=_f32, device=dev)
    dh0 = torch.empty(ndir, B, H, dtype=_f32, device=dev) if need_dh0 else None
    nbytes = _gru_ws_bytes('xps_gru_seq_bwd_f32_workspace', T, B, H, ndir)
    ws = _ws(nbytes, dev)
    _gru_status_register(dev)
    if split4:
        fused = drop is not None and dy is not None
        call('xps_gru_seq_bwd_split4_f32', _ptr(dy), _ptr(dhn), _ptr(y_ext), _ptr(saved), _ptr_array(w_hh), _ptr_array(w_t), _ptr(dgi),
             _ptr(dghn), _ptr(dh0), T, B, H, ndir, float(drop[0]) if fused else 0.0, int(drop[1]) if fused else 0, _ptr(ws), nbytes,
             _stream())
        return dgi, dghn, dh0
    if drop is not None and dy is not None:
        call('xps_gru_seq_bwd_drop_f32', _ptr(dy), _ptr(dhn), _ptr(y_ext), _ptr(saved), _ptr_array(w_hh), _ptr_array(w_t), _ptr(dgi),
             _ptr(dghn), _ptr(dh0), T, B, H, ndir, float(drop[0]), int(drop[1]), _ptr(ws), nbytes, _stream())
        return dgi, dghn, dh0
    call('xps_gru_seq_bwd_f32', _ptr(dy), _ptr(dhn), _ptr(y_ext), _ptr(saved), _ptr_array(w_hh), _ptr_array(w_t), _ptr(dgi),
         _ptr(dghn), _ptr(dh0), T, B, H, ndir, _ptr(ws), nbytes, _stream())
    return dgi, dghn, dh0


def _recurrent_grad_problems(dgi, dghn, y_ext, w_hh_params, b_hh_params, T, B, H, ndir, fmt=0, y_fmt=0):
    dev = y_ext.device
    ldy = ndir * H
    probs, rets = [], []
    for d in range(ndir):
        dw, db, acc_w, rw, rb = _grad_targets(w_hh_params[d], (3 * H, H), b_hh_params[d], (3 * H,), dev)
        first_slot = 0 if d == 0 else 2
        hprev = y_ext.view(-1)[first_slot * B * ldy + d * H:]
        probs.append(tn_problem(dgi[d], hprev, dw, 2 * H, H, T * B, ra=rowmap(3 * H, fmt=fmt), rb=rowmap(ldy, fmt=y_fmt), rc=rowmap(H),
                                colsum_out=db, accumulate=acc_w))
        probs.append(tn_problem(dghn[d], hprev, dw[2 * H:], H, H, T * B, ra=rowmap(H, fmt=fmt), rb=rowmap(ldy, fmt=y_fmt), rc=rowmap(H),
                                colsum_out=db[2 * H:], accumulate=acc_w))
        rets.append((rw, rb))
    return probs, rets


class GRURecurFn(torch.autograd.Function):

    @staticmethod
    def forward(ctx, gi, h0, ndir, *wb):
        _need_gpu(gi, h0, *wb)
        w_hh = [w.contiguous() for w in wb[:ndir]]
        b_hh = [b.contiguous() for b in wb[ndir:]]
        gi = gi.contiguous()
        _, T, B, H3 = gi.shape
        H = H3 // 3
        h0c = None if h0 is None else h0.contiguous()
        save = any(ctx.needs_input_grad)
        y_ext, saved = _gru_forward(gi, w_hh, b_hh, h0c, T, B, H, ndir, save)
        if save:
            ctx.save_for_backward(y_ext, saved, *w_hh)
            ctx.form = saved.launch_form
        ctx.params = wb
        ctx.dims = (T, B, H, ndir)
        ctx.has_h0 = h0 is not None
        return y_ext

    @staticmethod
    def backward(ctx, dy_ext):
        y_ext, saved, *w_hh = ctx.saved_tensors
        T, B, H, ndir = ctx.dims
        need_dh0 = ctx.has_h0 and ctx.needs_input_grad[1]
        dgi, dghn, dh0 = _gru_backward(dy_ext[1:T + 1], None, y_ext, saved, w_hh, T, B, H, ndir, need_dh0, form=ctx.form)
        if need_dh0:
            dh0[0] += dy_ext[0, :, :H]
            if ndir == 2:
                dh0[1] += dy_ext[T + 1, :, H:]
        probs, rets = _recurrent_grad_problems(dgi, dghn, y_ext, ctx.params[:ndir], ctx.params[ndir:], T, B, H, ndir)
        gemm_tn_grouped(probs, y_ext.device)
        return (dgi, dh0, None, *[r[0] for r in rets], *[r[1] for r in rets])


HN_NONE, HN_STACK, HN_SUM = 0, 1, 2


FMT_X_SPLIT4, FMT_Y_SPLIT4 = 1, 2


def split4_mode():
    return lib().xps_get_gemm_precision() == 1 and os.environ.get('XPS_SPLIT4', '1') != '0'


def layer_output_split4_ok(T, B, H, ndir, drop_p):
    return bool(drop_p and drop_p > 0.0 and split4_mode() and H > 256 and (ndir * H) % 4 == 0
                and not fused_dropout_supported(T, B, H, ndir))


def _presplit_weights_ok(rows, In, H3):
    return (split4_mode() and In % 4 == 0 and rows >= 4096 and In * H3 >= int(os.environ.get('XPS_SPLIT4_WEIGHTS_MIN', 1 << 19))
            and os.environ.get('XPS_SPLIT4_WEIGHTS', '1') != '0')


def skinny_dx_wanted(rows, In, K):
    return (os.environ.get('XPS_SKINNY_DX', '0') == '1' and split4_mode() and In % 4 == 0 and In < 256 and rows % 256 == 0
            and rows >= 96 * 256 and K % 32 == 0 and K >= 512 and os.environ.get('XPS_GEMM_DMA', '1') != '0')


def split4_pad(w, ldo):
    w = w.contiguous()
    out = torch.empty(w.shape[0], ldo, dtype=_f32, device=w.device)
    call('xps_split4_pad_f32', _ptr(w), w.shape[1], w.shape[0], w.shape[1], _ptr(out), ldo, _stream())
    return out


def split4(x, drop_p=0.0, seed=0):
    out = torch.empty_like(x)
    call('xps_split4_f32', _ptr(x), _ptr(out), x.numel(), float(drop_p), int(seed), _stream())
    return out


class GruPlan(NamedTuple):
    cluster_on: bool
    precision: int
    drop_fused: bool
    x_fmt: int
    w_fmt: int
    y_out_split: bool
    fwd_images: bool
    fwd_ysplit: bool
    want_dropped: bool
    bwd_split4: int
    y_fmt: int
    skinny_dx: bool


def gru_layer_plan(T, B, In, H, ndir, drop_p, fmt):
    has_drop = bool(drop_p and drop_p > 0.0)
    drop_fused = bool(has_drop and fused_dropout_supported(T, B, H, ndir))
    y_out_split = bool(fmt & FMT_Y_SPLIT4)
    if y_out_split and (not has_drop or drop_fused):
        raise ValueError('FMT_Y_SPLIT4: only with a separate dropout pass (see layer_output_split4_ok)')
    w_fmt = 1 if _presplit_weights_ok(T * B, In, 3 * H) else 0
    split4 = bool(split4_wanted(T, B, H, ndir))
    hprev = bool(hprev_split_wanted(T, B, H, ndir, split4))
    fwd_images = bool(fwd_images_wanted(T, B, H, ndir, hprev))
    return GruPlan(cluster_on=lib().xps_get_gru_cluster_mode() != 0, precision=lib().xps_get_gemm_precision(), drop_fused=drop_fused,
                   x_fmt=1 if (fmt & FMT_X_SPLIT4) else 0, w_fmt=w_fmt, y_out_split=y_out_split, fwd_images=fwd_images,
                   fwd_ysplit=bool(fwd_ysplit_wanted(T, B, H, ndir, hprev)), want_dropped=fwd_images and y_out_split,
                   bwd_split4=int(split4), y_fmt=int(hprev),
                   skinny_dx=bool(split4 and not w_fmt and skinny_dx_wanted(T * B, In, 3 * H)))


class GRULayerFmtFn(torch.autograd.Function):

    @staticmethod
    def forward(ctx, x, ndir, hn_mode, drop_p, fmt, *wb):
        ctx.set_materialize_grads(False)
        _need_gpu(x, *wb)
        x = x.contiguous()
        T, B, In = x.shape
        w_ih = [wb[4 * d + 0].contiguous() for d in range(ndir)]
        w_hh = [wb[4 * d + 1].contiguous() for d in range(ndir)]
        b_ih = [wb[4 * d + 2].contiguous() for d in range(ndir)]
        b_hh = [wb[4 * d + 3].contiguous() for d in range(ndir)]
        H = w_hh[0].shape[1]
        plan = ctx.plan = gru_layer_plan(T, B, In, H, ndir, drop_p, fmt)
        gi = torch.empty(ndir, T, B, 3 * H, dtype=_f32, device=x.device)
        if plan.w_fmt:
            w_ih = [split4(w) for w in w_ih]
        ra, rb, rc = rowmap(In, fmt=plan.x_fmt), rowmap(In, fmt=plan.w_fmt), rowmap(3 * H)
        call('xps_gemm_nt_multi_f32', _ptr(x), C.byref(ra), _ptr_array(w_ih), C.byref(rb), _ptr_array([gi[d] for d in range(ndir)]),
             C.byref(rc), _ptr_array(b_ih), ndir, T * B, 3 * H, In, _stream())
        save = any(ctx.needs_input_grad)
        drop = None
        y_drop = None
        if drop_p and drop_p > 0.0:
            drop = (float(drop_p), next_dropout_seed())
        ctx.drop = drop
        y_split = None
        if (save and (plan.fwd_images or plan.fwd_ysplit)) or plan.want_dropped:
            y_ext, saved, y_split, y_drop = _gru_forward_images(gi, w_hh, b_hh, T, B, H, ndir, save, plan.want_dropped, drop)
        elif plan.drop_fused:
            y_ext, saved, y_drop = _gru_forward(gi, w_hh, b_hh, None, T, B, H, ndir, save, drop)
        else:
            y_ext, saved = _gru_forward(gi, w_hh, b_hh, None, T, B, H, ndir, save)
        if save:
            ctx.save_for_backward(x, y_ext, saved, *w_ih, *w_hh, *([y_split] if y_split is not None else []))
        ctx.params = wb
        ctx.dims = (T, B, H, ndir, In, hn_mode)
        y = y_ext[1:T + 1]
        if y_drop is not None:
            y = y_drop
        elif drop is not None:
            out = torch.empty(T, B, ndir * H, dtype=_f32, device=x.device)
            if plan.y_out_split:
                call('xps_split4_f32', _ptr(y), _ptr(out), out.numel(), drop[0], drop[1], _stream())
            else:
                call('xps_dropout_f32', _ptr(y), _ptr(out), None, out.numel(), drop[0], drop[1], _stream())
            y = out
        if hn_mode == HN_NONE:
            hn = None
        elif hn_mode == HN_SUM:
            hn = y_ext[T, :, :H] + y_ext[1, :, H:] if ndir == 2 else y_ext[T, :, :H].clone()
        else:
            hn = torch.stack([y_ext[T, :, :H]] + ([y_ext[1, :, H:]] if ndir == 2 else []), dim=0)
        return y, hn

    @staticmethod
    def backward(ctx, dy, dhn):
        T, B, H, ndir, In, hn_mode = ctx.dims
        if dhn is not None and hn_mode == HN_SUM:
            dhn = dhn.unsqueeze(0).expand(ndir, B, H).contiguous()
        plan = ctx.plan
        if lib().xps_get_gemm_precision() != plan.precision:
            names = {v: k for k, v in GEMM_PRECISIONS.items()}
            raise RuntimeError(f'GRU backward: the forward chose its operand formats in {names[plan.precision]} mode but the backward '
                               f'runs in {names[lib().xps_get_gemm_precision()]} mode: the product precision (set_gemm_precision / '
                               'XPS_GEMM_PRECISION) must not change between a forward and its backward')
        x, y_ext, saved, *w = ctx.saved_tensors
        y_split = w.pop() if (plan.fwd_images or plan.fwd_ysplit) else None
        w_ih, w_hh = w[:ndir], w[ndir:]
        fmt, y_fmt, x_fmt, w_fmt = plan.bwd_split4, plan.y_fmt, plan.x_fmt, plan.w_fmt
        wb = ctx.params
        if ctx.drop is not None and dy is not None and not plan.drop_fused:
            dyc = dy.contiguous()
            dyd = torch.empty_like(dyc)
            call('xps_dropout_f32', _ptr(dyc), _ptr(dyd), None, dyc.numel(), ctx.drop[0], ctx.drop[1], _stream())
            dy = dyd
        dgi, dghn, _ = _gru_backward(dy, dhn, y_ext, saved, w_hh, T, B, H, ndir, False, ctx.drop if plan.drop_fused else None,
                                     split4=bool(fmt), form=(plan.cluster_on, B, H))
        dev = x.device
        have_img = y_split is not None
        y_src = (y_split if have_img else torch.empty_like(y_ext)) if y_fmt else y_ext
        probs, rets_hh = _recurrent_grad_problems(dgi, dghn, y_src, [wb[4 * d + 1] for d in range(ndir)],
                                                  [wb[4 * d + 3] for d in range(ndir)], T, B, H, ndir, fmt, y_fmt)
        rets_ih = []
        for d in range(ndir):
            dw, db, acc_w, rw, rb = _grad_targets(wb[4 * d + 0], (3 * H, In), wb[4 * d + 2], (3 * H,), dev)
            probs.append(tn_problem(dgi[d], x, dw, 3 * H, In, T * B, ra=rowmap(3 * H, fmt=fmt), rb=rowmap(In, fmt=x_fmt),
                                    colsum_out=db, accumulate=acc_w))
            rets_ih.append((rw, rb))
        direct = all(r[0] is None and r[1] is None for r in rets_ih + rets_hh)
        def launch_group(st):
            if y_fmt and not have_img:
                call('xps_split4_f32', _ptr(y_ext), _ptr(y_src), y_ext.numel(), 0.0, 0, _stream() if st is None else st)
            return gemm_tn_grouped(probs, dev, st)
        _launch_weight_grads(launch_group, dev, (dgi, dghn, x, y_ext, y_src), direct)
        dx = None
        if ctx.needs_input_grad[0]:
            dx = torch.empty(T, B, In, dtype=_f32, device=dev)
            if plan.skinny_dx:
                w_ih = [split4_pad(w, 256) for w in w_ih]
                w_fmt, ldw = 1, 256
            else:
                ldw = In
            if ndir == 2:
                ra, rb, rc = rowmap(3 * H, fmt=fmt), rowmap(ldw, fmt=w_fmt), rowmap(In)
                call('xps_gemm_nn2_f32', _ptr(dgi[0]), _ptr(w_ih[0]), 3 * H, _ptr(dgi[1]), _ptr(w_ih[1]), 3 * H,
                     C.byref(ra), C.byref(rb), _ptr(dx), C.byref(rc), T * B, In, 0, _stream())
            else:
                gemm_nn(dgi[0], w_ih[0], dx, T * B, In, 3 * H, ra=rowmap(3 * H, fmt=fmt), rb=rowmap(ldw, fmt=w_fmt))
        grads = []
        for d in range(ndir):
            grads += [rets_ih[d][0], rets_hh[d][0], rets_ih[d][1], rets_hh[d][1]]
        return (dx, None, None, None, None, *grads)


class GRULayerDropFn(torch.autograd.Function):

    @staticmethod
    def forward(ctx, x, ndir, hn_mode, drop_p, *wb):
        return GRULayerFmtFn.forward(ctx, x, ndir, hn_mode, drop_p, 0, *wb)

    @staticmethod
    def backward(ctx, dy, dhn):
        g = GRULayerFmtFn.backward(ctx, dy, dhn)
        return g[:4] + g[5:]


class GRULayerFn(torch.autograd.Function):

    @staticmethod
    def forward(ctx, x, ndir, hn_mode, *wb):
        return GRULayerDropFn.forward(ctx, x, ndir, hn_mode, 0.0, *wb)

    @staticmethod
    def backward(ctx, dy, dhn):
        g = GRULayerDropFn.backward(ctx, dy, dhn)
        return g[:3] + g[4:]


POST_SYNCBN_HOOKS = []
def _dp_world(group):
    import torch.distributed as dist
    if group is not None and dist.is_available() and dist.is_initialized():
        return dist.get_world_size(group)
    return 1


def _dp_enabled(group):
    return _dp_world(group) > 1


def _dist_sum_(t, group):
    if _dp_enabled(group):
        import torch.distributed as dist
        dist.all_reduce(t, op=dist.ReduceOp.SUM, group=group)
        return True
    return False


def _global_rows(rows, group, device, global_trials, Tp):
    if global_trials is not None:
        return float(global_trials) * Tp
    cnt = torch.tensor([float(rows)], dtype=torch.float64, device=device)
    _dist_sum_(cnt, group)
    return float(cnt.item())


class TemporalConvFn(torch.autograd.Function):

    @staticmethod
    def forward(ctx, x, conv_w, conv_b, gamma, beta, running_mean, running_var, stride, training,
                relu, drop_mask, drop_scale, momentum, eps, group, global_trials=None, num_batches_tracked=None):
        _need_gpu(x, conv_w)
        x = x.contiguous()
        B, T, Cin = x.shape
        F, _, k = conv_w.shape
        Tp = (T - k) // stride + 1
        if Tp < 1:
            raise ValueError('TemporalConv: sequence shorter than the kernel')
        w2 = conv_w.permute(0, 2, 1).contiguous().view(F, k * Cin)
        rows = Tp * B
        y = torch.empty(Tp, B, F, dtype=_f32, device=x.device)
        ra = rowmap(stride * Cin, rpg=Tp, gs=T * Cin)
        rc = rowmap(B * F, rpg=Tp, gs=F)
        gemm_nt(x, w2, y, rows, F, k * Cin, bias=conv_b, ra=ra, rc=rc)
        out = torch.empty_like(y)
        if training:
            stats = torch.empty(2 * F, dtype=_f32, device=x.device)
            nbytes = lib().xps_colsum_f32_workspace(rows, F)
            ws = _ws(nbytes, x.device)
            call('xps_colsum_f32', _ptr(y), F, rows, F, _ptr(stats), None, 0, _ptr(ws), nbytes, _stream())
            count = float(rows)
            if _dist_sum_(stats[:F], group):
                count = _global_rows(rows, group, x.device, global_trials, Tp)
            call('xps_bn_centered_sumsq_f32', _ptr(y), rows, F, _ptr(stats), count, _ptr(stats[F:]), _ptr(ws), nbytes,
                 _stream())
            _dist_sum_(stats[F:], group)
            mean = torch.empty(F, dtype=_f32, device=x.device)
            rstd = torch.empty(F, dtype=_f32, device=x.device)
            call('xps_bn_finalize_apply_f32', _ptr(y), _ptr(stats), count, _ptr(gamma), _ptr(beta), _ptr(mean), _ptr(rstd),
                 _ptr(running_mean), _ptr(running_var), _ptr(num_batches_tracked), momentum, eps, _ptr(drop_mask), drop_scale,
                 _ptr(out), rows, F, int(relu), _stream())
            ctx.save_for_backward(x, w2, y, out, mean, rstd, gamma, drop_mask)
            ctx.cfg = (B, T, Cin, F, k, stride, Tp, relu, drop_scale, count, group)
            ctx.conv_w = conv_w
            ctx.conv_b = conv_b
            ctx.bn_params = (gamma, beta)
        else:
            call('xps_bn_apply_eval_f32', _ptr(y), _ptr(running_mean), _ptr(running_var), eps, _ptr(gamma),
                 _ptr(beta), _ptr(out), rows, F, int(relu), _stream())
        return out

    @staticmethod
    def backward(ctx, dout):
        x, w2, y, out, mean, rstd, gamma, drop_mask = ctx.saved_tensors
        B, T, Cin, F, k, stride, Tp, relu, drop_scale, count, group = ctx.cfg
        rows = Tp * B
        dev = x.device
        dout = dout.contiguous()
        sums = torch.empty(2 * F, dtype=_f32, device=dev)
        nbytes = lib().xps_bn_bwd_workspace(rows, F)
        ws = _ws(nbytes, dev)
        g_beta, acc_beta, _ = _grad_target(ctx.bn_params[1], (F,), dev)
        g_gamma, acc_gamma, _ = _grad_target(ctx.bn_params[0], (F,), dev)
        direct_bn = acc_beta and acc_gamma
        dp = _dp_enabled(group)
        call('xps_bn_bwd_reduce_f32', _ptr(dout), _ptr(out), _ptr(y), _ptr(mean), _ptr(rstd), _ptr(drop_mask),
             drop_scale, int(relu), _ptr(sums), _ptr(g_beta) if direct_bn else None, _ptr(g_gamma) if direct_bn else None,
             rows, F, _ptr(ws), nbytes, _stream())
        dbeta = dgamma = None
        if not direct_bn:
            local = sums.clone() if dp else sums
            dbeta, dgamma = local[:F], local[F:]
        if dp:
            _dist_sum_(sums, group)
            for hook in list(POST_SYNCBN_HOOKS):
                hook()
        dy = torch.empty_like(y)
        call('xps_bn_bwd_apply_f32', _ptr(dout), _ptr(out), _ptr(y), _ptr(mean), _ptr(rstd), _ptr(gamma),
             _ptr(drop_mask), drop_scale, int(relu), _ptr(sums), count, _ptr(dy), rows, F, _stream())
        dconv_b, acc_cb, r_cb = _grad_target(ctx.conv_b, (F,), dev) if ctx.conv_b is not None else (None, False, None)
        if dconv_b is None:
            dconv_b = r_cb = torch.empty(F, dtype=_f32, device=dev)
        dw2 = torch.empty(F, k * Cin, dtype=_f32, device=dev)
        gemm_tn_grouped([tn_problem(dy, x, dw2, F, k * Cin, rows, ra=rowmap(F),
                                    rb=rowmap(T * Cin, rpg=B, gs=stride * Cin), colsum_out=dconv_b,
                                    accumulate_colsum=acc_cb)], dev)
        gw, acc_w, _ = _grad_target(ctx.conv_w, (F, Cin, k), dev)
        if acc_w:
            gw.add_(dw2.view(F, k, Cin).permute(0, 2, 1))
            dconv_w = None
        else:
            dconv_w = dw2.view(F, k, Cin).permute(0, 2, 1).contiguous()
        return (None, dconv_w, r_cb, dgamma, dbeta) + (None,) * 12


def decoder_supported(H, C, L):
    return bool(lib().xps_decoder_supported(int(H), int(C), int(L)))


class DecoderFn(torch.autograd.Function):

    @staticmethod
    def forward(ctx, table, h0, w_hh, b_hh, w_fc, b_fc, teacher, flags, start_token, L):
        ctx.set_materialize_grads(False)
        _need_gpu(table, h0, w_hh, w_fc)
        table, h0c = table.contiguous(), h0.contiguous()
        w_hh_c, b_hh_c, w_fc_c, b_fc_c = w_hh.contiguous(), b_hh.contiguous(), w_fc.contiguous(), b_fc.contiguous()
        B, H = h0c.shape
        C = w_fc_c.shape[0]
        ntok = table.shape[0]
        dev = h0c.device
        save = any(ctx.needs_input_grad)
        logits = torch.empty(B, L, C, dtype=_f32, device=dev)
        tokens = torch.empty(L, B, dtype=torch.int64, device=dev)
        hs = torch.empty(L + 1, B, H, dtype=_f32, device=dev)
        saved = torch.empty(L, B, 4 * H, dtype=_f32, device=dev) if save else None
        if teacher is not None:
# ... 638 lines not shown
```

### cross_patient_speech_decoding_amd/nn_models/models.py

```python
import os

import torch
import torch.nn as nn

from . import functional as XF
from ._lightning import LightningModule


def cmat_acc(y_hat, y, num_classes):
    y_pred = torch.argmax(y_hat, dim=1)
    cm = torch.bincount(y * num_classes + y_pred, minlength=num_classes * num_classes)
    cm = cm.view(num_classes, num_classes)
    return cm.diag().sum() / cm.sum()


class _HipCrossEntropyLoss(nn.CrossEntropyLoss):

    def forward(self, input, target):
        plain = (self.weight is None and self.reduction == 'mean' and self.ignore_index == -100
                 and self.label_smoothing == 0.0 and input.dim() == 2 and input.is_cuda)
        if plain:
            return XF.cross_entropy(input, target)
        return super().forward(input, target)


class BaseLightningModel(LightningModule):

    def __init__(self, criterion=None, learning_rate=1e-3, l2_reg=1e-5):
        super().__init__()
        self.criterion = criterion if criterion is not None else _HipCrossEntropyLoss()
        self.learning_rate = learning_rate
        self.l2_reg = l2_reg

    def _shared_step(self, batch, stage):
        x, y = batch
        y_hat = self(x)
        loss = self.criterion(y_hat, y)
        acc = cmat_acc(y_hat, y, self.num_classes)
        self.log_dict({f'{stage}_loss': loss, f'{stage}_acc': acc}, prog_bar=True)
        return loss

    def training_step(self, batch, batch_idx):
        return self._shared_step(batch, 'train')

    def validation_step(self, batch, batch_idx):
        return self._shared_step(batch, 'val')

    def test_step(self, batch, batch_idx):
        return self._shared_step(batch, 'test')

    def predict_step(self, batch, batch_idx):
        x, _ = batch
        return self(x)

    def configure_optimizers(self):
        return torch.optim.AdamW(self.parameters(), lr=self.learning_rate, weight_decay=self.l2_reg)


class TemporalConv(nn.Module):

    def __init__(self, in_channels, out_channels, kernel_size, stride=1, padding=0, dropout=0.2,
                 activation=True):
        super().__init__()
        self.conv = nn.Conv1d(in_channels, out_channels, kernel_size, stride=stride, padding=padding)
        self.bn = nn.BatchNorm1d(out_channels)
        self.relu = nn.ReLU()
        self.dropout = nn.Dropout(dropout)
        self.activation = activation
        self.process_group = None
        self.global_batch = None

    def forward_tm(self, x):
        k, s, pad = self.conv.kernel_size[0], self.conv.stride[0], self.conv.padding[0]
        if pad > 0:
            x = torch.nn.functional.pad(x, (0, 0, pad, pad))
        B, T, _ = x.shape
        Tp = (T - k) // s + 1
        F = self.conv.out_channels
        training = self.training
        mask, scale, p = None, 1.0, self.dropout.p
        if training and p > 0:
            mask = XF.dropout_mask((Tp, B, F), p, x.device)
            scale = 1.0 / (1.0 - p)
        momentum = 0.1 if self.bn.momentum is None else self.bn.momentum
        nbt = self.bn.num_batches_tracked if training and self.bn.track_running_stats else None
        return XF.TemporalConvFn.apply(x, self.conv.weight, self.conv.bias, self.bn.weight, self.bn.bias,
                                       self.bn.running_mean, self.bn.running_var, s, training,
                                       bool(self.activation), mask, scale, momentum, self.bn.eps,
                                       self.process_group, self.global_batch if self.process_group is not None else None,
                                       nbt)

    def forward(self, x):
        return self.forward_tm(x.permute(0, 2, 1)).permute(1, 2, 0)


def _gru_layer_weights(rnn, layer, ndir):
    out = []
    for d in range(ndir):
        sfx = f'_l{layer}' + ('_reverse' if d == 1 else '')
        out += [getattr(rnn, 'weight_ih' + sfx), getattr(rnn, 'weight_hh' + sfx),
                getattr(rnn, 'bias_ih' + sfx), getattr(rnn, 'bias_hh' + sfx)]
    return out


class EncoderRNN(nn.Module):

    def __init__(self, input_size, hidden_size, num_layers, dropout=0.3, model_type='gru'):
        super().__init__()
        self.model_type = model_type
        if model_type == 'gru':
            self.rnn = nn.GRU(input_size, hidden_size, num_layers, batch_first=True, dropout=dropout,
                              bidirectional=True)
        elif model_type == 'lstm':
            raise NotImplementedError("model_type='lstm' is not on the accelerated path (the reference's LSTM "
                                      'branch is itself broken: models.py:280 repeats a tuple)')
        else:
            raise ValueError('model_type must be one of "gru" or "lstm"')

    def forward_tm(self, x):
        y, last = self.forward_tm_last(x)
        return y, last.unsqueeze(0)

    def forward_tm_last(self, x):
        rnn = self.rnn
        L = rnn.num_layers
        y = x
        fmt = 0
        for l in range(L):
            p_drop = float(rnn.dropout) if (l < L - 1 and self.training) else 0.0
            T_, B_ = y.shape[0], y.shape[1]
            out_split = XF.layer_output_split4_ok(T_, B_, rnn.hidden_size, 2, p_drop)
            y, last = XF.GRULayerFmtFn.apply(y, 2, XF.HN_SUM if l == L - 1 else XF.HN_NONE, p_drop,
                                             fmt | (XF.FMT_Y_SPLIT4 if out_split else 0), *_gru_layer_weights(rnn, l, 2))
            fmt = XF.FMT_X_SPLIT4 if out_split else 0
        return y, last

    def forward(self, x):
        y, h = self.forward_tm(x.permute(1, 0, 2))
        return y.permute(1, 0, 2), h


class DecoderRNN(nn.Module):

    def __init__(self, hidden_size, output_size, num_layers, dropout=0.3, model_type='gru'):
        super().__init__()
        self.embedding = nn.Embedding(output_size + 1, hidden_size)
        if model_type != 'gru':
            raise NotImplementedError("model_type='lstm' is not on the accelerated path")
        self.rnn = nn.GRU(hidden_size, hidden_size, num_layers, batch_first=True, dropout=dropout)
        self.fc_out = nn.Linear(hidden_size, output_size)

    def token_projection(self):
        return XF.linear(self.embedding.weight, self.rnn.weight_ih_l0, self.rnn.bias_ih_l0)

    def step(self, tok, hidden, table):
        rnn = self.rnn
        B = tok.shape[0]
        H = rnn.hidden_size
        new_h = []
        gi = XF.gather_rows(table, tok).view(1, 1, B, 3 * H)
        y_ext = XF.GRURecurFn.apply(gi, hidden[0:1], 1, rnn.weight_hh_l0, rnn.bias_hh_l0)
        h = y_ext[1]
        new_h.append(h)
        for l in range(1, rnn.num_layers):
            inp = XF.dropout(h, rnn.dropout, self.training)
            gi = XF.linear(inp, getattr(rnn, f'weight_ih_l{l}'), getattr(rnn, f'bias_ih_l{l}')).view(1, 1, B, 3 * H)
            y_ext = XF.GRURecurFn.apply(gi, hidden[l:l + 1], 1, getattr(rnn, f'weight_hh_l{l}'),
                                        getattr(rnn, f'bias_hh_l{l}'))
            h = y_ext[1]
            new_h.append(h)
        logits = XF.linear(h, self.fc_out.weight, self.fc_out.bias)
        return logits, torch.stack(new_h, dim=0)

    def forward(self, x, hidden):
        return self.step(x, hidden, self.token_projection())


class Seq2SeqRNN(BaseLightningModel):

    def __init__(self, in_channels, n_filters, hidden_size, num_classes, n_enc_layers, n_dec_layers,
                 kernel_size, stride=1, padding=0, cnn_dropout=0.3, rnn_dropout=0.3, model_type='gru',
                 learning_rate=1e-3, l2_reg=1e-5, criterion=None, activation=True, seq_length=3,
                 decay_iters=20):
        super().__init__(learning_rate=learning_rate, l2_reg=l2_reg, criterion=criterion)
        self.num_classes = num_classes
        self.seq_length = seq_length
        self.temporal_conv = TemporalConv(in_channels, n_filters, kernel_size, stride, padding, cnn_dropout,
                                          activation=activation)
        self.encoder = EncoderRNN(n_filters, hidden_size, n_enc_layers, dropout=rnn_dropout,
                                  model_type=model_type)
        self.decoder = DecoderRNN(hidden_size, num_classes, n_dec_layers, dropout=rnn_dropout,
                                  model_type=model_type)
        self.decay_iters = decay_iters

    def draw_teacher_coins(self, y, teacher_forcing_ratio):
        coins = []
        for _ in range(self.seq_length):
            coins.append(bool(y is not None and torch.rand(1).item() < teacher_forcing_ratio))
        return coins

    def forward(self, x, y=None, teacher_forcing_ratio=0.5, coins=None):
        if coins is None:
            coins = self.draw_teacher_coins(y, teacher_forcing_ratio)
        return self.forward_device(x, y, self._device_flags(tuple(bool(c) and y is not None for c in coins), x.device))

    def _device_flags(self, bits, device):
        cache = self.__dict__.setdefault('_flag_cache', {})
        key = (bits, device)
        t = cache.get(key)
        if t is None:
            t = torch.tensor([int(b) for b in bits], dtype=torch.int32).to(device)
            if len(cache) < 4096:
                cache[key] = t
        return t

    def forward_device(self, x, y, flags):
        z = self.temporal_conv.forward_tm(x)
        _, enc_last = self.encoder.forward_tm_last(z)
        rnn = self.decoder.rnn
        if (rnn.num_layers == 1 and self.num_classes + 1 <= 16
                and XF.decoder_supported(rnn.hidden_size, self.num_classes, self.seq_length)):
            table = self.decoder.token_projection()
            logits, _ = XF.DecoderFn.apply(table, enc_last, rnn.weight_hh_l0, rnn.bias_hh_l0,
                                           self.decoder.fc_out.weight, self.decoder.fc_out.bias,
                                           y if y is not None else None, flags if y is not None else None,
                                           self.num_classes, self.seq_length)
            return logits
        if rnn.num_layers == 1 and rnn.hidden_size % 4 == 0 and os.environ.get('XPS_DECODER_WIDE', '1') != '0':
            table = self.decoder.token_projection()
            logits, _ = XF.DecoderWideFn.apply(table, enc_last, rnn.weight_hh_l0, rnn.bias_hh_l0,
                                               self.decoder.fc_out.weight, self.decoder.fc_out.bias,
                                               y if y is not None else None, flags if y is not None else None,
                                               self.num_classes, self.seq_length)
            return logits
        dec_hidden = enc_last.unsqueeze(0).repeat(self.decoder.rnn.num_layers, 1, 1)
        B = x.size(0)
        tok = torch.full((B,), self.num_classes, dtype=torch.long, device=x.device)
        table = self.decoder.token_projection()
        outputs = []
        for i in range(self.seq_length):
            logits, dec_hidden = self.decoder.step(tok, dec_hidden, table)
            outputs.append(logits)
            if i + 1 < self.seq_length:
                teacher = y[:, i] if y is not None else None
                tok = XF.next_token(logits.detach(), teacher, flags[i:i + 1] if y is not None else None)
        return torch.stack(outputs, dim=1)

    def _seq_step(self, batch, stage, ratio):
        x, y = batch
        y_hat = self(x, y, teacher_forcing_ratio=ratio).view(-1, self.num_classes)
        y = y.reshape(-1)
        loss = self.criterion(y_hat, y)
        acc = cmat_acc(y_hat, y, self.num_classes)
        self.log_dict({f'{stage}_loss': loss, f'{stage}_acc': acc}, prog_bar=True)
        return loss

    def training_step(self, batch, batch_idx):
        return self._seq_step(batch, 'train', 0.5)

    def validation_step(self, batch, batch_idx):
        return self._seq_step(batch, 'val', 0)

    def test_step(self, batch, batch_idx):
        return self._seq_step(batch, 'test', 0)

    def configure_optimizers(self):
        optim = torch.optim.AdamW(self.parameters(), lr=self.learning_rate, weight_decay=self.l2_reg)
        lr_sch = torch.optim.lr_scheduler.LinearLR(optim, start_factor=1.0, end_factor=0.01,
                                                   total_iters=self.decay_iters)
        return {'optimizer': optim, 'lr_scheduler': {'scheduler': lr_sch, 'interval': 'epoch', 'frequency': 1}}


def _plain_hip_criterion(criterion):
    return (type(criterion) is _HipCrossEntropyLoss and criterion.weight is None and criterion.reduction == 'mean'
            and criterion.ignore_index == -100 and criterion.label_smoothing == 0.0)


class _ClassifyStepMixin:

    def _classify_step(self, batch, stage):
        x, y = batch
        y_hat = self(x)
        if _plain_hip_criterion(self.criterion) and y_hat.is_cuda and y_hat.dim() == 2:
            loss, acc, _ = XF.classify_loss_acc(y_hat, y, self.num_classes)
        else:
            loss = self.criterion(y_hat, y)
            acc = cmat_acc(y_hat, y, self.num_classes)
        self.log_dict({f'{stage}_loss': loss, f'{stage}_acc': acc}, prog_bar=True)
        return loss

    def training_step(self, batch, batch_idx):
        return self._classify_step(batch, 'train')

    def validation_step(self, batch, batch_idx):
        return self._classify_step(batch, 'val')

    def test_step(self, batch, batch_idx):
        return self._classify_step(batch, 'test')


def _fc_stack(dim_fc, num_classes):
    return nn.Sequential(*[nn.Linear(dim_fc[i], dim_fc[i + 1]) for i in range(len(dim_fc) - 1)]
                         + [nn.Linear(dim_fc[-1], num_classes)])


def _apply_fc(fc, x):
    if fc is None:
        return x
    for lin in (fc if isinstance(fc, nn.Sequential) else [fc]):
        x = XF.linear(x, lin.weight, lin.bias)
    return x


class SimpleGRU(nn.Module):

    def __init__(self, input_size, hidden_size, out_size, num_layers, dropout=0.3, bidir=False):
        super().__init__()
        if bidir:
            raise NotImplementedError('SimpleGRU(bidir=True): the reference module cannot run it either (its Linear takes '
                                      'hidden_size inputs, a bidirectional GRU emits 2 * hidden_size)')
        self.gru = nn.GRU(input_size, hidden_size, num_layers, batch_first=True, bidirectional=False, dropout=dropout)
        self.fc = nn.Linear(hidden_size, out_size)

    def forward_tm(self, z):
        rnn = self.gru
        L = rnn.num_layers
        y, hn = z, None
        for l in range(L):
            p_drop = float(rnn.dropout) if (l < L - 1 and self.training) else 0.0
            y, hn = XF.GRULayerFmtFn.apply(y, 1, XF.HN_SUM if l == L - 1 else XF.HN_NONE, p_drop, 0,
                                           *_gru_layer_weights(rnn, l, 1))
        return XF.linear(hn, self.fc.weight, self.fc.bias)

    def forward(self, x):
        return self.forward_tm(x.permute(1, 0, 2))


class TemporalConvRNN(_ClassifyStepMixin, BaseLightningModel):

    def __init__(self, in_channels, n_filters, num_classes, hidden_size, n_layers, kernel_size, dim_fc=None, stride=1,
                 padding=0, cnn_dropout=0.3, rnn_dropout=0.3, learning_rate=1e-3, l2_reg=1e-5, criterion=None,
                 activation=True, decay_iters=20):
        super().__init__(learning_rate=learning_rate, l2_reg=l2_reg, criterion=criterion)
        self.num_classes = num_classes
        self.decay_iters = decay_iters
        self.temporal_conv = TemporalConv(in_channels, n_filters, kernel_size, stride, padding, cnn_dropout,
                                          activation=activation)
        if dim_fc is None:
            self.rnn = SimpleGRU(n_filters, hidden_size, num_classes, n_layers, dropout=rnn_dropout)
            self.fc = None
        elif isinstance(dim_fc, list):
            self.rnn = SimpleGRU(n_filters, hidden_size, dim_fc[0], n_layers, dropout=rnn_dropout)
            self.fc = _fc_stack(dim_fc, num_classes)
        else:
            self.rnn = SimpleGRU(n_filters, hidden_size, dim_fc, n_layers, dropout=rnn_dropout)
            self.fc = nn.Linear(dim_fc, num_classes)

    def forward(self, x):
        z = self.temporal_conv.forward_tm(x)
        return _apply_fc(self.fc, self.rnn.forward_tm(z))

    def configure_optimizers(self):
        optim = torch.optim.AdamW(self.parameters(), lr=self.learning_rate, weight_decay=self.l2_reg)
        lr_sch = torch.optim.lr_scheduler.LinearLR(optim, start_factor=1.0, end_factor=0.01,
                                                   total_iters=self.decay_iters)
        return {'optimizer': optim, 'lr_scheduler': {'scheduler': lr_sch, 'interval': 'epoch', 'frequency': 1}}


class TCN_classifier(_ClassifyStepMixin, BaseLightningModel):

    def __init__(self, in_channels, num_classes, dim_fc, kernel_size, stride=1, padding=0, dropout=0.3,
                 learning_rate=1e-3, l2_reg=1e-5, criterion=None, activation=True):
        super().__init__(learning_rate=learning_rate, l2_reg=l2_reg, criterion=criterion)
        self.num_classes = num_classes
        n_filters = dim_fc[0] if isinstance(dim_fc, list) else dim_fc
        self.temporal_conv = TemporalConv(in_channels, n_filters, kernel_size, stride, padding, dropout,
                                          activation=activation)
        if isinstance(dim_fc, list):
            self.fc = _fc_stack(dim_fc, num_classes)
        else:
            self.fc = nn.Linear(dim_fc, num_classes)

    def forward(self, x):
        z = self.temporal_conv.forward_tm(x)
        return _apply_fc(self.fc, XF.time_max(z))


class PositionalEncoding(nn.Module):

    def __init__(self, d_model, max_len=5000):
        super().__init__()
        dim = d_model + (d_model % 2)
        enc = torch.zeros(max_len, dim)
        position = torch.arange(0, max_len, dtype=torch.float).unsqueeze(1)
        div_term = torch.exp(torch.arange(0, dim, 2).float() * (-torch.log(torch.tensor(10000.0)) / dim))
        enc[:, 0::2] = torch.sin(position * div_term)
        enc[:, 1::2] = torch.cos(position * div_term)
        self.register_buffer('pos_encoding', enc.unsqueeze(0)[:, :, :d_model])

    def forward_tm(self, z, batch_major=False):
        S = z.shape[1] if batch_major else z.shape[0]
        if S > self.pos_encoding.shape[1]:
            raise ValueError(f'PositionalEncoding: sequence length {S} exceeds max_len {self.pos_encoding.shape[1]}')
        return XF.add_positional(z, self.pos_encoding[0], batch_major)

    def forward(self, x):
        return self.forward_tm(x, batch_major=True).permute(1, 0, 2)


class CosineWarmupScheduler(torch.optim.lr_scheduler._LRScheduler):

    def __init__(self, optimizer, warmup, max_iters):
        self.warmup = warmup
        self.max_num_iters = max_iters
        super().__init__(optimizer)

    def get_lr(self):
        lr_factor = self.get_lr_factor(epoch=self.last_epoch)
        return [base_lr * lr_factor for base_lr in self.base_lrs]

    def get_lr_factor(self, epoch):
        import numpy as np
        lr_factor = 0.5 * (1 + np.cos(np.pi * epoch / self.max_num_iters))
        if epoch <= self.warmup:
            lr_factor *= epoch * 1.0 / self.warmup
        return lr_factor


def _make_encoder(d_model, n_head, dim_fc, dropout, num_layers):
    XF.check_attention_shape(d_model, n_head)
    layer = nn.TransformerEncoderLayer(d_model, n_head, dim_fc, dropout, batch_first=True)
    return nn.TransformerEncoder(layer, num_layers, enable_nested_tensor=False)


def _encoder_stack_tm(encoder, z, training):
    S, B, D = z.shape
    x = z.reshape(S * B, D)
    for layer in encoder.layers:
        att = layer.self_attn
        if layer.norm_first or getattr(layer, 'activation_relu_or_gelu', 1) != 1:
            raise NotImplementedError('the HIP encoder layer is post-norm with ReLU (the reference\'s configuration)')
        qkv = XF.linear(x, att.in_proj_weight, att.in_proj_bias)
        ctx = XF.self_attention(qkv, B, S, att.num_heads, att.dropout, training)
        a = XF.linear(ctx, att.out_proj.weight, att.out_proj.bias)
        x = XF.add_layer_norm(x, a, layer.norm1.weight, layer.norm1.bias, layer.norm1.eps, layer.dropout1.p, training)
        h = XF.relu_dropout(XF.linear(x, layer.linear1.weight, layer.linear1.bias), layer.dropout.p, training)
        f = XF.linear(h, layer.linear2.weight, layer.linear2.bias)
        x = XF.add_layer_norm(x, f, layer.norm2.weight, layer.norm2.bias, layer.norm2.eps, layer.dropout2.p, training)
    if encoder.norm is not None:
        raise NotImplementedError('a final encoder norm is not part of the reference\'s models')
    return x.view(S, B, D)


class Transformer(_ClassifyStepMixin, BaseLightningModel):

    def __init__(self, in_channels, num_classes, d_model, kernel_size, stride=1, padding=0, n_head=8, num_layers=3, dim_fc=128,
                 dropout=0.3, learning_rate=1e-3, l2_reg=1e-5, criterion=None):
        super().__init__(learning_rate=learning_rate, l2_reg=l2_reg, criterion=criterion)
        self.num_classes = num_classes
        self.positional_encoding = PositionalEncoding(d_model)
        self.transformer_encoder = _make_encoder(d_model, n_head, dim_fc, dropout, num_layers)
        self.fc = nn.Linear(d_model, num_classes)

    def forward(self, x):
        z = self.positional_encoding.forward_tm(x, batch_major=True)
        z = _encoder_stack_tm(self.transformer_encoder, z, self.training)
        return XF.linear(XF.time_mean(z), self.fc.weight, self.fc.bias)


class CNNTransformer(_ClassifyStepMixin, BaseLightningModel):

    def __init__(self, in_channels, num_classes, d_model, kernel_size, stride=1, padding=0, n_head=8, num_layers=3, dim_fc=128,
                 cnn_dropout=0.2, transformer_dropout=0.3, learning_rate=1e-3, warmup=20, max_epochs=500, l2_reg=1e-5,
                 criterion=None, activation=True):
        super().__init__(learning_rate=learning_rate, l2_reg=l2_reg, criterion=criterion)
        self.num_classes = num_classes
        self.temporal_conv = TemporalConv(in_channels, d_model, kernel_size, stride, padding, cnn_dropout, activation=activation)
        self.positional_encoding = PositionalEncoding(d_model)
        self.transformer_encoder = _make_encoder(d_model, n_head, dim_fc, transformer_dropout, num_layers)
        self.fc = nn.Linear(d_model, num_classes)
        self.warmup = warmup
        self.max_epochs = max_epochs

# ... 15 lines not shown
```

### include/xps.h

```cpp
#ifndef XPS_H
#define XPS_H

#include <stddef.h>
#include <stdint.h>

#ifdef __cplusplus
extern "C" {
#endif

#define XPS_OK 0
#define XPS_E_INVALID (-1)
#define XPS_E_HIP (-2)
#define XPS_E_WORKSPACE (-3)

typedef struct xps_rowmap {
    int64_t gs;
    int64_t ld;
    int32_t rpg;
    int32_t fmt;
} xps_rowmap;
#define XPS_FMT_F32 0
#define XPS_FMT_SPLIT4 1

const char* xps_last_error(void);
int xps_abi_version(void);
int xps_stream_create_low_priority(void** stream);
int xps_stream_destroy(void* stream);
int xps_set_gemm_precision(int mode);
int xps_get_gemm_precision(void);
int xps_set_gemm_big_tiles(int on);
int xps_get_gemm_big_tiles(void);


int xps_gemm_nt_f32(const float* A, const xps_rowmap* ra, const float* B, const xps_rowmap* rb,
                    float* C, const xps_rowmap* rc, const float* bias,
                    int M, int N, int K, int accumulate, void* stream);
int xps_gemm_nn_f32(const float* A, const xps_rowmap* ra, const float* B, const xps_rowmap* rb,
                    float* C, const xps_rowmap* rc,
                    int M, int N, int K, int accumulate, void* stream);
int xps_gemm_nt_multi_f32(const float* A, const xps_rowmap* ra, const float* const* B, const xps_rowmap* rb,
                          float* const* C, const xps_rowmap* rc, const float* const* bias, int nprob,
                          int M, int N, int K, void* stream);
int xps_gemm_nn2_f32(const float* A1, const float* B1, int K1, const float* A2, const float* B2, int K2,
                     const xps_rowmap* ra, const xps_rowmap* rb, float* C, const xps_rowmap* rc,
                     int M, int N, int accumulate, void* stream);
size_t xps_gemm_tn_f32_workspace(int M, int N, int K);
int xps_gemm_tn_f32(const float* A, const xps_rowmap* ra, const float* B, const xps_rowmap* rb,
                    float* C, const xps_rowmap* rc,
                    int M, int N, int K, int accumulate,
                    void* workspace, size_t workspace_bytes, void* stream);

typedef struct xps_tn_problem {
    const float* A; const float* B; float* C; float* colsum_a;
    xps_rowmap ra, rb, rc;
    int32_t M, N, K, accumulate;
} xps_tn_problem;
size_t xps_gemm_tn_grouped_f32_workspace(const xps_tn_problem* probs, int n);
int xps_gemm_tn_grouped_f32(const xps_tn_problem* probs, int n, void* workspace, size_t workspace_bytes,
                            void* stream);

size_t xps_colsum_f32_workspace(int rows, int cols);
int xps_colsum_f32(const float* X, int64_t ldx, int rows, int cols, float* out, float* out_sq,
                   int accumulate, void* workspace, size_t workspace_bytes, void* stream);

size_t xps_gru_seq_fwd_f32_workspace(int T, int B, int H, int ndir);
long long xps_gru_seq_status_offset(int T, int B, int H, int ndir);
int xps_gru_set_status_word(unsigned* device_word);
int xps_set_gru_bptt_grid(int two_dimensional);
int xps_get_gru_bptt_grid(void);
int xps_set_gru_cluster_mode(int mode);
int xps_get_gru_cluster_mode(void);
int xps_gru_seq_fwd_f32(const float* gi, const float* const* w_hh, const float* const* b_hh,
                        const float* h0, float* y_ext, float* saved,
                        int T, int B, int H, int ndir, void* workspace, size_t workspace_bytes, void* stream);

size_t xps_gru_seq_bwd_f32_workspace(int T, int B, int H, int ndir);
int xps_gru_seq_bwd_f32(const float* dy, const float* dhn, const float* y_ext, const float* saved,
                        const float* const* w_hh, const float* const* w_hh_t, float* dgi, float* dghn, float* dh0,
                        int T, int B, int H, int ndir, void* workspace, size_t workspace_bytes, void* stream);
int xps_gru_seq_fused_dropout_supported(int T, int B, int H, int ndir);
int xps_gru_seq_fwd_drop_f32(const float* gi, const float* const* w_hh, const float* const* b_hh,
                             const float* h0, float* y_ext, float* saved,
                             int T, int B, int H, int ndir, float* y_drop, float drop_p, uint64_t drop_seed,
                             void* workspace, size_t workspace_bytes, void* stream);
int xps_gru_seq_bwd_drop_f32(const float* dy, const float* dhn, const float* y_ext, const float* saved,
                             const float* const* w_hh, const float* const* w_hh_t, float* dgi, float* dghn, float* dh0,
                             int T, int B, int H, int ndir, float drop_p, uint64_t drop_seed,
                             void* workspace, size_t workspace_bytes, void* stream);
int xps_gru_seq_fwd_images_supported(int T, int B, int H, int ndir);
int xps_gru_seq_fwd_image_exchange_supported(int T, int B, int H, int ndir);
int xps_gru_seq_fwd_images_f32(const float* gi, const float* const* w_hh, const float* const* b_hh,
                               const float* h0, float* y_ext, float* saved, int T, int B, int H, int ndir,
                               float* y_split, float* y_drop_split, float drop_p, uint64_t drop_seed,
                               void* workspace, size_t workspace_bytes, void* stream);
int xps_gru_seq_bwd_split4_supported(int T, int B, int H, int ndir);
int xps_gru_seq_bwd_split4_f32(const float* dy, const float* dhn, const float* y_ext, const float* saved,
                               const float* const* w_hh, const float* const* w_hh_t, float* dgi, float* dghn, float* dh0,
                               int T, int B, int H, int ndir, float drop_p, uint64_t drop_seed,
                               void* workspace, size_t workspace_bytes, void* stream);

int xps_transpose_f32(const float* src, float* dst, int rows, int cols, void* stream);
int xps_transpose_batched_f32(const float* const* src, float* const* dst, int n, int rows, int cols, void* stream);

int xps_bn_centered_sumsq_f32(const float* y, int rows, int F, const float* stats, double count, float* out_sq,
                              void* workspace, size_t workspace_bytes, void* stream);
int xps_bn_finalize_f32(const float* stats, double count, float* mean, float* rstd,
                        float* running_mean, float* running_var, int64_t* num_batches_tracked,
                        float momentum, float eps, int F, void* stream);
int xps_bn_apply_f32(const float* y, const float* mean, const float* rstd,
                     const float* gamma, const float* beta, const float* drop_mask, float drop_scale,
                     float* out, int64_t rows, int F, int relu, void* stream);
int xps_bn_finalize_apply_f32(const float* y, const float* stats, double count, const float* gamma, const float* beta,
                              float* mean, float* rstd, float* running_mean, float* running_var,
                              int64_t* num_batches_tracked, float momentum, float eps, const float* drop_mask,
                              float drop_scale, float* out, int64_t rows, int F, int relu, void* stream);
int xps_bn_apply_eval_f32(const float* y, const float* running_mean, const float* running_var, float eps,
                          const float* gamma, const float* beta, float* out,
                          int64_t rows, int F, int relu, void* stream);
size_t xps_bn_bwd_workspace(int64_t rows, int F);
int xps_bn_bwd_reduce_f32(const float* dout, const float* out, const float* y, const float* mean,
                          const float* rstd, const float* drop_mask, float drop_scale, int relu,
                          float* sums, float* dbeta_acc, float* dgamma_acc, int64_t rows, int F,
                          void* workspace, size_t workspace_bytes, void* stream);
int xps_bn_bwd_apply_f32(const float* dout, const float* out, const float* y, const float* mean,
                         const float* rstd, const float* gamma, const float* drop_mask,
                         float drop_scale, int relu, const float* sums, double count,
                         float* dy, int64_t rows, int F, void* stream);

int xps_decoder_supported(int H, int C, int L);
int xps_decoder_fwd_f32(const float* table, const float* w_hh, const float* b_hh, const float* h0,
                        const float* w_fc, const float* b_fc, const int64_t* teacher, const int32_t* flags,
                        float* logits, int64_t* tokens, float* hs, float* saved,
                        int B, int H, int C, int L, int ntok, int start_token, void* stream);
int xps_decoder_bwd_f32(const float* dlogits, const float* hs, const float* saved, const float* w_hh_t,
                        const float* w_fc, float* dgi, float* dghn, float* dh0,
                        int B, int H, int C, int L, void* stream);

int xps_gemv_f32(const float* x, const float* W, const float* bias, float* out, int N, int K, int B,
                 void* stream);
int xps_gru_cell_gemv_f32(const float* x, int K, const float* w_ih, const float* w_hh, const float* b_ih,
                          const float* b_hh, const float* h_prev, float* h_new, int H, int B, void* stream);

int xps_window_shift_f32(const double* power, int k, int C, const double* W, const double* c, const float* src,
                         float* dst, int win, int d, int B, void* stream);
int xps_ctc_collapse_f32(const float* logits, int n_classes, int blank, int64_t* argmax, int32_t* state,
                         int64_t* tokens, int max_tokens, int B, void* stream);

size_t xps_ctc_beam_workspace(int B, int T, int beam_size, int n_classes);
int xps_ctc_beam_f64(const void* log_probs, int is_f32, int B, int T, int n_classes, const int64_t* input_lengths,
                     int blank, int beam_size, int from_logits, int64_t* prefix, int64_t* prefix_len, double* nll,
                     void* workspace, size_t workspace_bytes, void* stream);
size_t xps_ctc_beam_state_bytes(int n_streams, int beam_size, int max_steps);
int xps_ctc_beam_step_f32(const float* logits, int n_classes, int blank, int beam_size, int max_steps, void* state,
                          size_t state_bytes, int B, void* stream);
int xps_ctc_beam_readout(const void* state, size_t state_bytes, int B, int beam_size, int max_steps, int s,
                         int64_t* prefix, int64_t* prefix_len, double* nll, void* stream);

int xps_gather_rows_f32(const float* table, const int64_t* idx, float* out,
                        int B, int cols, int n_rows, void* stream);
size_t xps_scatter_rows_f32_workspace(int B, int cols, int n_rows);
int xps_scatter_rows_f32(const float* dout, const int64_t* idx, float* dtable,
                         int B, int cols, int n_rows, int accumulate,
                         void* workspace, size_t workspace_bytes, void* stream);
int xps_next_token(const float* logits, int n_classes, const int64_t* teacher, int64_t teacher_stride,
                   const int32_t* use_teacher, int64_t* next, int B, void* stream);
int xps_decoder_select_f32(const float* h, const float* w_fc, const float* b_fc, float* logits,
                           const int64_t* teacher, int64_t teacher_stride, const int32_t* use_teacher,
                           const float* table, int64_t* next, float* gi_next, int B, int H, int C, int ntok, void* stream);
int xps_dropout_f32(const float* x, float* out, float* mask, int64_t n, float p, uint64_t seed, void* stream);
int xps_split4_f32(const float* x, float* out, int64_t n, float drop_p, uint64_t seed, void* stream);
int xps_split4_pad_f32(const float* x, int64_t ldx, int rows, int cols, float* out, int64_t ldo, void* stream);
int xps_mask_scale_f32(const float* x, const float* mask, float scale, float* out, int64_t n, void* stream);
int xps_add_f32(const float* a, const float* b, float* out, int64_t n, void* stream);

int xps_cross_entropy_fwd_f32(const float* logits, const int64_t* target, float* row_loss,
                              float* loss, int64_t rows, int n_classes, void* stream);
int xps_cross_entropy_bwd_f32(const float* logits, const int64_t* target, const float* gout,
                              float* dlogits, int64_t rows, int n_classes, void* stream);
size_t xps_cross_entropy_loss_grad_f32_workspace(int64_t rows);
int xps_cross_entropy_loss_grad_f32(const float* logits, const int64_t* target, float* row_loss, float* loss,
                                    float* dlogits, void* workspace, size_t workspace_bytes, int64_t rows,
                                    int n_classes, void* stream);
size_t xps_classify_loss_acc_f32_workspace(int64_t rows);
int xps_classify_loss_acc_f32(const float* logits, const int64_t* target, float* row_loss, float* loss, float* dlogits,
                              int64_t* cmat, float* acc, void* workspace, size_t workspace_bytes, int64_t rows,
                              int n_classes, void* stream);
int xps_time_max_fwd_f32(const float* z, float* out, int* arg, int T, int B, int F, void* stream);
int xps_time_max_bwd_f32(const float* dout, const int* arg, float* dz, int T, int B, int F, void* stream);

int xps_attention_supported(int B, int S, int n_head, int dh);
int xps_attention_fwd_f32(const float* qkv, float* ctx, float* lse, int B, int S, int n_head, int dh, float p, uint64_t seed,
                          void* stream);
size_t xps_attention_bwd_f32_workspace(int B, int S, int n_head, int dh);
int xps_attention_bwd_f32(const float* dctx, const float* qkv, const float* ctx, const float* lse, float* dqkv, int B, int S,
                          int n_head, int dh, float p, uint64_t seed, void* workspace, size_t workspace_bytes, void* stream);
int xps_add_layer_norm_fwd_f32(const float* x, const float* r, const float* gamma, const float* beta, float* y, float* mean,
                               float* rstd, int64_t rows, int D, float eps, float p, uint64_t seed, void* stream);
size_t xps_add_layer_norm_bwd_f32_workspace(int64_t rows, int D);
// ... 119 lines not shown
```

Measured before the change: 328,200 trials/s.

## Fuse inter-layer dropout backward mask into next layer's dx GEMM epilogue

Adds a dropout-mask epilogue to the GEMM kernels and a new nn2_drop entry point. The next GRU layer's input-gradient GEMM now applies the previous layer's dropout mask as it stores, through a DropLink/DropSite handoff between layers. This removes a separate elementwise dropout pass over dy in the previous layer's backward, when that layer's dropout was not already fused. It adds template variants, cross-layer state coupling and a runtime check, and it only fires when dropout is unfused and the skinny dx path is not taken.

```diff
diff --git a/cross_patient_speech_decoding_amd/csrc/xps_common.h b/cross_patient_speech_decoding_amd/csrc/xps_common.h
--- a/cross_patient_speech_decoding_amd/csrc/xps_common.h
+++ b/cross_patient_speech_decoding_amd/csrc/xps_common.h
@@ -49,13 +49,22 @@
 
 __device__ inline float sigmoidf_acc(float x) { return 1.0f / (1.0f + expf(-x)); }
 
-__device__ inline void rng_pair(unsigned long long seed, long long pair, float& u0, float& u1) {
-    unsigned long long z = seed + 0x9E3779B97F4A7C15ull * (unsigned long long)(pair + 1);
+constexpr unsigned long long RNG_STRIDE = 0x9E3779B97F4A7C15ull;
+__device__ inline void rng_mix_bits(unsigned long long z, unsigned& k0, unsigned& k1) {
     z = (z ^ (z >> 30)) * 0xBF58476D1CE4E5B9ull;
     z = (z ^ (z >> 27)) * 0x94D049BB133111EBull;
     z ^= z >> 31;
-    u0 = (float)((unsigned)(z >> 40)) * (1.0f / 16777216.0f);
-    u1 = (float)((unsigned)(z >> 8) & 0xFFFFFFu) * (1.0f / 16777216.0f);
+    k0 = (unsigned)(z >> 40);
+    k1 = (unsigned)(z >> 8) & 0xFFFFFFu;
+}
+__device__ inline void rng_mix(unsigned long long z, float& u0, float& u1) {
+    unsigned k0, k1;
+    rng_mix_bits(z, k0, k1);
+    u0 = (float)k0 * (1.0f / 16777216.0f);
+    u1 = (float)k1 * (1.0f / 16777216.0f);
+}
+__device__ inline void rng_pair(unsigned long long seed, long long pair, float& u0, float& u1) {
+    rng_mix(seed + RNG_STRIDE * (unsigned long long)(pair + 1), u0, u1);
 }
 __device__ inline f32x4 split4_pack(const f32x4 v) {
     typedef __bf16 bf16x8_ __attribute__((ext_vector_type(8)));
@@ -74,5 +83,19 @@
     rng_pair(seed, 2 * q + 1, u2, u3);
     return (f32x4){u0 >= p ? 1.f : 0.f, u1 >= p ? 1.f : 0.f, u2 >= p ? 1.f : 0.f, u3 >= p ? 1.f : 0.f};
 }
+__device__ inline float dropout_keep1(unsigned long long seed, long long i, float p) {
+    float u0, u1;
+    rng_pair(seed, i >> 1, u0, u1);
+    return ((i & 1) ? u1 : u0) >= p ? 1.f : 0.f;
+}
+
+struct DropEpi {
+    unsigned long long seed;
+    long long base;
+    float p, scale;
+};
+__device__ inline float lane_xor1(float v) {
+    return __builtin_bit_cast(float, __builtin_amdgcn_update_dpp(0, __builtin_bit_cast(int, v), 0xB1, 0xF, 0xF, true));
+}
 
 int xps_internal_gemm_mode();
diff --git a/cross_patient_speech_decoding_amd/csrc/xps_gemm.hip b/cross_patient_speech_decoding_amd/csrc/xps_gemm.hip
--- a/cross_patient_speech_decoding_amd/csrc/xps_gemm.hip
+++ b/cross_patient_speech_decoding_amd/csrc/xps_gemm.hip
@@ -14,12 +14,12 @@
 #ifndef XPS_BF_MI1_WAVES
 #define XPS_BF_MI1_WAVES XPS_GEMM_WAVES
 #endif
-template <bool AK, bool BK, int MI, bool EDGE = false, bool BF = false, bool PRE = false>
+template <bool AK, bool BK, int MI, bool EDGE = false, bool BF = false, bool PRE = false, bool DROP = false>
 __global__ __launch_bounds__(256, (BF && MI == 1) ? XPS_BF_MI1_WAVES : XPS_GEMM_WAVES) void gemm_f32_kernel(
     const float* __restrict__ A, RowMap ra, const float* __restrict__ B, RowMap rb,
     const float* __restrict__ A2, const float* __restrict__ B2, int K2,
     float* __restrict__ C, RowMap rc, const float* __restrict__ bias,
-    int M, int N, int K, int kchunk, long long slab_stride, int accumulate, int vecA, int vecB) {
+    int M, int N, int K, int kchunk, long long slab_stride, int accumulate, int vecA, int vecB, DropEpi drop) {
     __shared__ __attribute__((aligned(16))) TileMem<BF, MI> mem;
     const int tiles_n = (N + BN - 1) / BN, tiles = tiles_n * ((M + 64 * MI - 1) / (64 * MI));
     const int lid = xcd_remap(blockIdx.x, gridDim.x);
@@ -33,7 +33,15 @@
     f32x4 nocs4 = {0.f, 0.f, 0.f, 0.f};
     gemm_accumulate_any<AK, BK, MI, EDGE, BF, PRE>(acc, nocs, nocs4, false, A, ra, B, rb, M, N, K, m0, n0, kbeg, kend, vecA, vecB, mem);
     if (A2) gemm_accumulate_any<AK, BK, MI, EDGE, BF, PRE>(acc, nocs, nocs4, false, A2, ra, B2, rb, M, N, K2, m0, n0, 0, K2, vecA, vecB, mem);
-    gemm_store<MI>(acc, C + (long long)z * slab_stride, rc, bias, M, N, m0, n0, accumulate);
+    if constexpr (DROP) gemm_store_drop<MI>(acc, C, rc.ld, M, N, m0, n0, drop);
+    else gemm_store<MI>(acc, C + (long long)z * slab_stride, rc, bias, M, N, m0, n0, accumulate);
+}
+
+__global__ void drop_rows_kernel(float* __restrict__ C, long long ldc, int M, int N, DropEpi d) {
+    const long long e = (long long)blockIdx.x * blockDim.x + threadIdx.x;
+    if (e >= (long long)M * N) return;
+    const long long o = (e / N) * ldc + e % N;
+    C[o] = (C[o] * dropout_keep1(d.seed, d.base + o, d.p)) * d.scale;
 }
 
 constexpr int SM_MAXM = 16, SM_SLICES = 16, SM_KC = 1024;
@@ -491,11 +499,11 @@
     }
 }
 
-template <bool AK, bool BK, bool DEEP, int FMT = 0>
+template <bool AK, bool BK, bool DEEP, int FMT = 0, bool DROP = false>
 __global__ __launch_bounds__(512, 1) void gemm_big_kernel(const float* __restrict__ A, long long lda, const float* __restrict__ B,
                                                            long long ldb, const float* __restrict__ A2, const float* __restrict__ B2,
                                                            int K2, float* __restrict__ C, long long ldc,
-                                                           const float* __restrict__ bias, int N, int K, int accumulate, int fmt) {
+                                                           const float* __restrict__ bias, int N, int K, int accumulate, int fmt, DropEpi drop) {
     const int tiles_n = FMT == 5 ? 1 : N / xps_big::TN;
     const int lid = xcd_remap(blockIdx.x, gridDim.x);
     const int m0 = (lid / tiles_n) * xps_big::TM, n0 = (lid % tiles_n) * xps_big::TN;
@@ -506,7 +514,8 @@
         const bool act = (int)((threadIdx.x >> 6) & 3) * 64 < N;
         xps_big::direct_dma_pipeline<!BK>(acc, A, lda, B, ldb, m0, 0, 0, K / 32, big_smem, act);
         if (A2) xps_big::direct_dma_pipeline<!BK>(acc, A2, lda, B2, ldb, m0, 0, 0, K2 / 32, big_smem, act);
-        xps_big::big_store_c_masked(acc, C, ldc, bias, m0, N, accumulate);
+        if constexpr (DROP) xps_big::big_store_c_masked_drop(acc, C, ldc, m0, N, drop);
+        else xps_big::big_store_c_masked(acc, C, ldc, bias, m0, N, accumulate);
         return;
     }
     if constexpr (FMT == 4) {
@@ -516,7 +525,8 @@
         big_accumulate<AK, BK, DEEP, DEEP ? -1 : FMT>(acc, nocs, false, A, lda, B, ldb, m0, n0, 0, K, !DEEP && (fmt & 1) != 0, !DEEP && (fmt & 2) != 0);
         if (A2) big_accumulate<AK, BK, DEEP, DEEP ? -1 : FMT>(acc, nocs, false, A2, lda, B2, ldb, m0, n0, 0, K2, !DEEP && (fmt & 1) != 0, !DEEP && (fmt & 2) != 0);
     }
-    xps_big::big_store_c(acc, C, ldc, bias, m0, n0, accumulate);
+    if constexpr (DROP) xps_big::big_store_c_drop(acc, C, ldc, m0, n0, drop);
+    else xps_big::big_store_c(acc, C, ldc, bias, m0, n0, accumulate);
 }
 
 template <bool DEEP, bool DMA = false>
@@ -697,9 +707,9 @@
     return (int)(mb * xps_big::TM);
 }
 
-template <bool AK, bool BK>
+template <bool AK, bool BK, bool DROP = false>
 int launch_gemm(const float* A, const RowMap& ra, const float* B, const RowMap& rb, const float* A2, const float* B2, int K2,
-                float* C, const RowMap& rc, const float* bias, int M, int N, int K, int accumulate, hipStream_t st) {
+                float* C, const RowMap& rc, const float* bias, int M, int N, int K, int accumulate, hipStream_t st, DropEpi drop = {}) {
     const int kchunk = ((K + BKT - 1) / BKT) * BKT + BKT;
     int vecA = (int)(map_vec_ok(A, ra) && (!A2 || map_vec_ok(A2, ra)));
     int vecB = (int)(map_vec_ok(B, rb) && (!B2 || map_vec_ok(B2, rb)));
@@ -712,6 +722,8 @@
     if (M <= SM_MAXM) {
         hipLaunchKernelGGL((gemm_small_kernel<AK, BK>), dim3(cdiv(N, 64)), dim3(1024), 0, st, A, ra, B, rb, A2, B2, K2, C, rc,
                            bias, M, N, K, accumulate, vecB);
+        if constexpr (DROP)
+            hipLaunchKernelGGL(drop_rows_kernel, dim3(cdiv((long long)M * N, 256)), dim3(256), 0, st, C, rc.ld, M, N, drop);
         return hipGetLastError() == hipSuccess ? 0 : -1;
     }
     if constexpr (AK && !BK) {
@@ -719,10 +731,10 @@
             M / xps_big::TM >= 96 && K % 32 == 0 && K2 % 32 == 0 && K + K2 >= 512 && big_plain(A, ra, M) && big_plain(B, rb, K) &&
             (!A2 || (big_plain(A2, ra, M) && big_plain(B2, rb, K2))) && rc.rpg >= M) {
             constexpr int lds = xps_big::direct_dma_lds<true>();
-            static const bool ready5 = big_prepare(gemm_big_kernel<true, false, false, 5>, lds);
+            static const bool ready5 = big_prepare(gemm_big_kernel<true, false, false, 5, DROP>, lds);
             if (ready5) {
-                hipLaunchKernelGGL((gemm_big_kernel<true, false, false, 5>), dim3(M / xps_big::TM), dim3(xps_big::NTHR), lds, st,
-                                   A, ra.ld, B, rb.ld, A2, B2, K2, C, rc.ld, bias, N, K, accumulate, fmt);
+                hipLaunchKernelGGL((gemm_big_kernel<true, false, false, 5, DROP>), dim3(M / xps_big::TM), dim3(xps_big::NTHR), lds, st,
+                                   A, ra.ld, B, rb.ld, A2, B2, K2, C, rc.ld, bias, N, K, accumulate, fmt, drop);
                 return hipGetLastError() == hipSuccess ? 0 : -1;
             }
         }
@@ -731,9 +743,9 @@
         (long long)(M / xps_big::TM) * (N / xps_big::TN) >= big_min_tiles() &&
         big_plain(A, ra, AK ? M : K) && big_plain(B, rb, BK ? N : K) && (!A2 || (big_plain(A2, ra, AK ? M : K2) && big_plain(B2, rb, BK ? N : K2))) &&
         rc.rpg >= M) {
-        static const bool ready = big_prepare(gemm_big_kernel<AK, BK, false, 0>, BIG_LDS) && big_prepare(gemm_big_kernel<AK, BK, false, 1>, BIG_LDS) &&
-                                  big_prepare(gemm_big_kernel<AK, BK, false, 2>, BIG_LDS) && big_prepare(gemm_big_kernel<AK, BK, false, 3>, BIG_LDS) &&
-                                  big_prepare(gemm_big_kernel<AK, BK, true>, BIG_LDS32);
+        static const bool ready = big_prepare(gemm_big_kernel<AK, BK, false, 0, DROP>, BIG_LDS) && big_prepare(gemm_big_kernel<AK, BK, false, 1, DROP>, BIG_LDS) &&
+                                  big_prepare(gemm_big_kernel<AK, BK, false, 2, DROP>, BIG_LDS) && big_prepare(gemm_big_kernel<AK, BK, false, 3, DROP>, BIG_LDS) &&
+                                  big_prepare(gemm_big_kernel<AK, BK, true, 0, DROP>, BIG_LDS32);
         if (ready) {
             const int Mfull = M;
             M = big_split_rows(M, N / xps_big::TN);
@@ -743,36 +755,38 @@
                 if (Mtail <= 0) return 0;
                 const float* At = AK ? A + (long long)M * ra.ld : A + M;
                 const float* A2t = A2 ? (AK ? A2 + (long long)M * ra.ld : A2 + M) : nullptr;
-                return launch_gemm<AK, BK>(At, ra, B, rb, A2t, B2, K2, C + (long long)M * rc.ld, rc, bias, Mtail, N, K, accumulate, st);
+                DropEpi dt = drop;
+                dt.base += (long long)M * rc.ld;
+                return launch_gemm<AK, BK, DROP>(At, ra, B, rb, A2t, B2, K2, C + (long long)M * rc.ld, rc, bias, Mtail, N, K, accumulate, st, dt);
             };
             bool dma_done = false;
             if constexpr (AK) {
                 if (fmt == 3 && K % 32 == 0 && K2 % 32 == 0 && dma_enabled()) {
                     constexpr int lds = xps_big::direct_dma_lds<!BK>();
-                    static const bool ready4 = big_prepare(gemm_big_kernel<AK, BK, false, 4>, lds);
+                    static const bool ready4 = big_prepare(gemm_big_kernel<AK, BK, false, 4, DROP>, lds);
                     if (ready4) {
-                        hipLaunchKernelGGL((gemm_big_kernel<AK, BK, false, 4>), bgrid, dim3(xps_big::NTHR), lds, st,
-                                           A, ra.ld, B, rb.ld, A2, B2, K2, C, rc.ld, bias, N, K, accumulate, fmt);
+                        hipLaunchKernelGGL((gemm_big_kernel<AK, BK, false, 4, DROP>), bgrid, dim3(xps_big::NTHR), lds, st,
+                                           A, ra.ld, B, rb.ld, A2, B2, K2, C, rc.ld, bias, N, K, accumulate, fmt, drop);
                         dma_done = true;
                     }
                 }
             }
             if (dma_done) {
             } else if (big_deep_allowed() && K % 32 == 0 && K2 % 32 == 0 && fmt == 0)
-                hipLaunchKernelGGL((gemm_big_kernel<AK, BK, true>), bgrid, dim3(xps_big::NTHR), BIG_LDS32, st,
-                                   A, ra.ld, B, rb.ld, A2, B2, K2, C, rc.ld, bias, N, K, accumulate, fmt);
+                hipLaunchKernelGGL((gemm_big_kernel<AK, BK, true, 0, DROP>), bgrid, dim3(xps_big::NTHR), BIG_LDS32, st,
+                                   A, ra.ld, B, rb.ld, A2, B2, K2, C, rc.ld, bias, N, K, accumulate, fmt, drop);
             else if (fmt == 0)
-                hipLaunchKernelGGL((gemm_big_kernel<AK, BK, false, 0>), bgrid, dim3(xps_big::NTHR), BIG_LDS, st,
-                                   A, ra.ld, B, rb.ld, A2, B2, K2, C, rc.ld, bias, N, K, accumulate, fmt);
+                hipLaunchKernelGGL((gemm_big_kernel<AK, BK, false, 0, DROP>), bgrid, dim3(xps_big::NTHR), BIG_LDS, st,
+                                   A, ra.ld, B, rb.ld, A2, B2, K2, C, rc.ld, bias, N, K, accumulate, fmt, drop);
             else if (fmt == 1)
-                hipLaunchKernelGGL((gemm_big_kernel<AK, BK, false, 1>), bgrid, dim3(xps_big::NTHR), BIG_LDS, st,
-                                   A, ra.ld, B, rb.ld, A2, B2, K2, C, rc.ld, bias, N, K, accumulate, fmt);
+                hipLaunchKernelGGL((gemm_big_kernel<AK, BK, false, 1, DROP>), bgrid, dim3(xps_big::NTHR), BIG_LDS, st,
+                                   A, ra.ld, B, rb.ld, A2, B2, K2, C, rc.ld, bias, N, K, accumulate, fmt, drop);
             else if (fmt == 2)
-                hipLaunchKernelGGL((gemm_big_kernel<AK, BK, false, 2>), bgrid, dim3(xps_big::NTHR), BIG_LDS, st,
-                                   A, ra.ld, B, rb.ld, A2, B2, K2, C, rc.ld, bias, N, K, accumulate, fmt);
+                hipLaunchKernelGGL((gemm_big_kernel<AK, BK, false, 2, DROP>), bgrid, dim3(xps_big::NTHR), BIG_LDS, st,
+                                   A, ra.ld, B, rb.ld, A2, B2, K2, C, rc.ld, bias, N, K, accumulate, fmt, drop);
             else
-                hipLaunchKernelGGL((gemm_big_kernel<AK, BK, false, 3>), bgrid, dim3(xps_big::NTHR), BIG_LDS, st,
-                                   A, ra.ld, B, rb.ld, A2, B2, K2, C, rc.ld, bias, N, K, accumulate, fmt);
+                hipLaunchKernelGGL((gemm_big_kernel<AK, BK, false, 3, DROP>), bgrid, dim3(xps_big::NTHR), BIG_LDS, st,
+                                   A, ra.ld, B, rb.ld, A2, B2, K2, C, rc.ld, bias, N, K, accumulate, fmt, drop);
             if (hipGetLastError() != hipSuccess) return -1;
             return run_tail();
         }
@@ -780,11 +794,11 @@
 #define XPS_LAUNCH_GEMM(MI_, EDGE_, BF_)                                                                              \
     do {                                                                                                              \
         if (BF_ && fmt)                                                                                               \
-            hipLaunchKernelGGL((gemm_f32_kernel<AK, BK, MI_, EDGE_, BF_, BF_>), grid, dim3(256), 0, st, A, ra, B, rb, A2, B2, K2, C, rc, \
-                               bias, M, N, K, kchunk, 0LL, accumulate, vecA, vecB);                                   \
+            hipLaunchKernelGGL((gemm_f32_kernel<AK, BK, MI_, EDGE_, BF_, BF_, DROP>), grid, dim3(256), 0, st, A, ra, B, rb, A2, B2, K2, C, rc, \
+                               bias, M, N, K, kchunk, 0LL, accumulate, vecA, vecB, drop);                                \
         else                                                                                                          \
-            hipLaunchKernelGGL((gemm_f32_kernel<AK, BK, MI_, EDGE_, BF_>), grid, dim3(256), 0, st, A, ra, B, rb, A2, B2, K2, C, rc, \
-                               bias, M, N, K, kchunk, 0LL, accumulate, vecA, vecB);                                   \
+            hipLaunchKernelGGL((gemm_f32_kernel<AK, BK, MI_, EDGE_, BF_, false, DROP>), grid, dim3(256), 0, st, A, ra, B, rb, A2, B2, K2, C, rc, \
+                               bias, M, N, K, kchunk, 0LL, accumulate, vecA, vecB, drop);                                \
     } while (0)
     const bool bf = bf_mode();
     if (use_small_tiles(M, N, K + K2)) {
@@ -970,6 +984,32 @@
     return XPS_OK;
 }
 
+extern "C" int xps_gemm_nn2_drop_f32(const float* A1, const float* B1, int K1, const float* A2, const float* B2, int K2,
+                                     const xps_rowmap* ra_, const xps_rowmap* rb_, float* C, const xps_rowmap* rc_,
+                                     int M, int N, int accumulate, float drop_p, uint64_t drop_seed, void* stream) {
+    XPS_CHECK_ARG(A1 && B1 && C && ra_ && rb_ && rc_, "null argument");
+    XPS_CHECK_ARG((A2 == nullptr) == (B2 == nullptr), "A2 and B2 must both be given or both NULL");
+    XPS_CHECK_ARG(M >= 0 && N >= 0 && K1 >= 0 && K2 >= 0, "negative size");
+    XPS_CHECK_ARG(drop_p >= 0.f && drop_p < 1.f, "drop_p must be in [0, 1)");
+    XPS_CHECK_ARG(accumulate == 0, "the dropout epilogue masks what it stores: accumulate must be 0");
+    if (M == 0 || N == 0) return XPS_OK;
+    RowMap ra = to_rowmap(ra_), rb = to_rowmap(rb_), rc = to_rowmap(rc_);
+    XPS_CHECK_ARG(rc.rpg >= M, "the dropout epilogue needs a plain C (rc.rpg >= M): the decision index is m * rc.ld + n");
+    if (!A2) K2 = 0;
+    const DropEpi drop = {(unsigned long long)drop_seed, 0LL, drop_p, 1.0f / (1.0f - drop_p)};
+    const int lrc = drop_p > 0.f ? launch_gemm<true, false, true>(A1, ra, B1, rb, A2, B2, K2, C, rc, nullptr, M, N, K1, 0, (hipStream_t)stream, drop)
+                                 : launch_gemm<true, false>(A1, ra, B1, rb, A2, B2, K2, C, rc, nullptr, M, N, K1, 0, (hipStream_t)stream);
+    if (lrc == -2) {
+        xps_set_error("xps_gemm_nn2_drop_f32: XPS_FMT_SPLIT4 operand needs bf16x3 mode, M > 16, 16-byte aligned rows and a contiguous extent that is a multiple of 4");
+        return XPS_E_INVALID;
+    }
+    if (lrc) {
+        xps_set_error("xps_gemm_nn2_drop_f32: launch failed: %s", hipGetErrorString(hipGetLastError()));
+        return XPS_E_HIP;
+    }
+    return XPS_OK;
+}
+
 extern "C" size_t xps_gemm_tn_f32_workspace(int M, int N, int K) {
     if (M <= 0 || N <= 0 || K <= 0) return 16;
     int s = tn_splits(M, N, K);
@@ -1001,11 +1041,11 @@
     if (bf_mode())
         hipLaunchKernelGGL((gemm_f32_kernel<false, false, 2, true, true>), grid, dim3(256), 0, (hipStream_t)stream,
                            A, ra, B, rb, (const float*)nullptr, (const float*)nullptr, 0, slabs, rs, (const float*)nullptr,
-                           M, N, K, kchunk, slab_stride, 0, (int)map_vec_ok(A, ra), (int)map_vec_ok(B, rb));
+                           M, N, K, kchunk, slab_stride, 0, (int)map_vec_ok(A, ra), (int)map_vec_ok(B, rb), DropEpi{});
     else
         hipLaunchKernelGGL((gemm_f32_kernel<false, false, 2>), grid, dim3(256), 0, (hipStream_t)stream,
                            A, ra, B, rb, (const float*)nullptr, (const float*)nullptr, 0, slabs, rs, (const float*)nullptr,
-                           M, N, K, kchunk, slab_stride, 0, (int)map_vec_ok(A, ra), (int)map_vec_ok(B, rb));
+                           M, N, K, kchunk, slab_stride, 0, (int)map_vec_ok(A, ra), (int)map_vec_ok(B, rb), DropEpi{});
     XPS_CHECK_LAUNCH();
     long long total = (long long)M * N;
     hipLaunchKernelGGL(splitk_reduce_kernel, dim3(cdiv(total, RED_OUT)), dim3(256), 0, (hipStream_t)stream,
diff --git a/cross_patient_speech_decoding_amd/csrc/xps_gemm_big.h b/cross_patient_speech_decoding_amd/csrc/xps_gemm_big.h
--- a/cross_patient_speech_decoding_amd/csrc/xps_gemm_big.h
+++ b/cross_patient_speech_decoding_amd/csrc/xps_gemm_big.h
@@ -331,6 +331,36 @@
         }
 }
 
+__device__ inline void big_store_c_drop(const f32x16 (&acc)[4][2], float* __restrict__ C, long long ldc, int m0, int n0, const DropEpi d) {
+    const int lane = threadIdx.x & 63, wave = threadIdx.x >> 6;
+    const int wm = (wave >> 2) * 128, wn = (wave & 3) * 64;
+    const int li = lane & 31, lk = lane >> 5;
+    const long long off = (long long)(m0 + wm + 4 * lk) * ldc + n0 + wn + li;
+    xps_tile::store_tiles_drop<4>(acc, C + off, d.base + off, ldc, d);
+}
+__device__ inline void big_store_c_masked_drop(const f32x16 (&acc)[4][2], float* __restrict__ C, long long ldc, int m0, int nvalid, const DropEpi d) {
+    const int lane = threadIdx.x & 63, wave = threadIdx.x >> 6;
+    const int wm = (wave >> 2) * 128, wn = (wave & 3) * 64;
+    const int li = lane & 31, lk = lane >> 5;
+    if (wn >= nvalid) return;
+    const long long off = (long long)(m0 + wm + 4 * lk) * ldc + wn + li;
+    float* cbase = C + off;
+    const long long fbase = d.base + off;
+    const bool ok[2] = {wn + li < nvalid, wn + 32 + li < nvalid};
+#pragma unroll
+    for (int i = 0; i < 4; ++i)
+#pragma unroll
+        for (int r = 0; r < 16; ++r) {
+            const long long ro = (long long)(i * 32 + (r & 3) + 8 * (r >> 2)) * ldc;
+#pragma unroll
+            for (int j = 0; j < 2; ++j) {
+                if (!ok[j]) continue;
+                const float k = dropout_keep1(d.seed, fbase + ro + j * 32, d.p);
+                __builtin_nontemporal_store(((acc[i][j][r] + 0.f) * k) * d.scale, &cbase[ro + j * 32]);
+            }
+        }
+}
+
 __device__ inline void big_slab_store(const f32x16 (&acc)[4][2], float* const (&sub)[4]) {
     const int lane = threadIdx.x & 63, wave = threadIdx.x >> 6;
     float* base = sub[(wave >> 2) * 2 + ((wave & 3) >> 1)] + lane * 4;
diff --git a/cross_patient_speech_decoding_amd/csrc/xps_gemm_tile.h b/cross_patient_speech_decoding_amd/csrc/xps_gemm_tile.h
--- a/cross_patient_speech_decoding_amd/csrc/xps_gemm_tile.h
+++ b/cross_patient_speech_decoding_amd/csrc/xps_gemm_tile.h
@@ -525,6 +525,80 @@
     }
 }
 
+template <int NI>
+__device__ inline void store_tiles_drop(const f32x16 (&acc)[NI][2], float* __restrict__ cbase, long long fbase, long long ldc, const DropEpi d) {
+    if (((fbase - (threadIdx.x & 31)) | ldc) & 1) {
+#pragma unroll
+        for (int i = 0; i < NI; ++i)
+#pragma unroll
+            for (int r = 0; r < 16; ++r) {
+                const long long ro = (long long)(i * 32 + (r & 3) + 8 * (r >> 2)) * ldc;
+#pragma unroll
+                for (int j = 0; j < 2; ++j)
+                    __builtin_nontemporal_store(((acc[i][j][r] + 0.f) * dropout_keep1(d.seed, fbase + ro + j * 32, d.p)) * d.scale, &cbase[ro + j * 32]);
+            }
+        return;
+    }
+    const bool odd = (threadIdx.x & 1) != 0;
+    const long long g = odd ? fbase + ldc - 1 : fbase;
+    const unsigned long long S = RNG_STRIDE * (unsigned long long)(ldc >> 1);
+    unsigned long long zi = d.seed + RNG_STRIDE * (unsigned long long)((g >> 1) + 1);
+    const unsigned thr = (unsigned)ceilf(d.p * 16777216.0f);
+#pragma unroll
+    for (int i = 0; i < NI; ++i) {
+        unsigned long long zq = zi;
+#pragma unroll
+        for (int q = 0; q < 4; ++q) {
+#pragma unroll
+            for (int h = 0; h < 2; ++h) {
+                const int r = 4 * q + 2 * h;
+                const long long ro = (long long)(i * 32 + 2 * h + 8 * q) * ldc;
+#pragma unroll
+                for (int j = 0; j < 2; ++j) {
+                    unsigned k0, k1;
+                    rng_mix_bits(zq + (h ? 2 * S : 0ull) + (j ? 16 * RNG_STRIDE : 0ull), k0, k1);
+                    const float f0 = k0 >= thr ? d.scale : 0.f, f1 = k1 >= thr ? d.scale : 0.f;
+                    const float got = lane_xor1(odd ? f0 : f1);
+                    const float fa = odd ? got : f0, fb = odd ? f1 : got;
+                    __builtin_nontemporal_store(acc[i][j][r] * fa, &cbase[ro + j * 32]);
+                    __builtin_nontemporal_store(acc[i][j][r + 1] * fb, &cbase[ro + ldc + j * 32]);
+                }
+            }
+            zq += 8 * S;
+        }
+        zi += 32 * S;
+    }
+}
+
+template <int MI>
+__device__ inline void gemm_store_drop(const f32x16 (&acc)[MI][2], float* __restrict__ C, long long ldc, int M, int N, int m0, int n0,
+                                       const DropEpi d) {
+    const int lane = threadIdx.x & 63, wave = threadIdx.x >> 6;
+    const int wm = (wave >> 1) * (32 * MI), wn = (wave & 1) * 64;
+    const int li = lane & 31, lk = lane >> 5;
+    if (m0 + 64 * MI <= M && n0 + 128 <= N) {
+        const long long off = (long long)(m0 + wm + 4 * lk) * ldc + n0 + wn + li;
+        store_tiles_drop<MI>(acc, C + off, d.base + off, ldc, d);
+        return;
+    }
+    const int c0 = n0 + wn + li, c1 = c0 + 32;
+#pragma unroll
+    for (int i = 0; i < MI; ++i) {
+#pragma unroll
+        for (int r = 0; r < 16; ++r) {
+            const int row = m0 + wm + i * 32 + (r & 3) + 8 * (r >> 2) + 4 * lk;
+            if (row >= M) continue;
+            const long long ro = (long long)row * ldc;
+#pragma unroll
+            for (int j = 0; j < 2; ++j) {
+                const int col = j ? c1 : c0;
+                if (col < N)
+                    __builtin_nontemporal_store(((acc[i][j][r] + 0.f) * dropout_keep1(d.seed, d.base + ro + col, d.p)) * d.scale, &C[ro + col]);
+            }
+        }
+    }
+}
+
 template <int MI>
 __device__ inline void zero_acc(f32x16 (&acc)[MI][2]) {
 #pragma unroll
diff --git a/cross_patient_speech_decoding_amd/nn_models/functional.py b/cross_patient_speech_decoding_amd/nn_models/functional.py
--- a/cross_patient_speech_decoding_amd/nn_models/functional.py
+++ b/cross_patient_speech_decoding_amd/nn_models/functional.py
@@ -472,9 +472,27 @@
     bwd_split4: int
     y_fmt: int
     skinny_dx: bool
-
-
-def gru_layer_plan(T, B, In, H, ndir, drop_p, fmt):
+    dx_drop: bool = False
+
+
+class DropSite:
+    __slots__ = ('p', 'seed', 'fused', 'y_ptr', 'y_shape', 'dx', 'applied')
+
+    def __init__(self, p, seed, fused, y):
+        self.p, self.seed, self.fused = p, seed, fused
+        self.y_ptr, self.y_shape = y.data_ptr(), tuple(y.shape)
+        self.dx = None
+        self.applied = False
+
+
+class DropLink:
+    __slots__ = ('site',)
+
+    def __init__(self):
+        self.site = None
+
+
+def gru_layer_plan(T, B, In, H, ndir, drop_p, fmt, site=None, need_dx=True):
     has_drop = bool(drop_p and drop_p > 0.0)
     drop_fused = bool(has_drop and fused_dropout_supported(T, B, H, ndir))
     y_out_split = bool(fmt & FMT_Y_SPLIT4)
@@ -484,17 +502,18 @@
     split4 = bool(split4_wanted(T, B, H, ndir))
     hprev = bool(hprev_split_wanted(T, B, H, ndir, split4))
     fwd_images = bool(fwd_images_wanted(T, B, H, ndir, hprev))
+    skinny = bool(split4 and not w_fmt and skinny_dx_wanted(T * B, In, 3 * H))
     return GruPlan(cluster_on=lib().xps_get_gru_cluster_mode() != 0, precision=lib().xps_get_gemm_precision(), drop_fused=drop_fused,
                    x_fmt=1 if (fmt & FMT_X_SPLIT4) else 0, w_fmt=w_fmt, y_out_split=y_out_split, fwd_images=fwd_images,
                    fwd_ysplit=bool(fwd_ysplit_wanted(T, B, H, ndir, hprev)), want_dropped=fwd_images and y_out_split,
-                   bwd_split4=int(split4), y_fmt=int(hprev),
-                   skinny_dx=bool(split4 and not w_fmt and skinny_dx_wanted(T * B, In, 3 * H)))
+                   bwd_split4=int(split4), y_fmt=int(hprev), skinny_dx=skinny,
+                   dx_drop=bool(site is not None and not site.fused and not skinny and need_dx))
 
 
 class GRULayerFmtFn(torch.autograd.Function):
 
     @staticmethod
-    def forward(ctx, x, ndir, hn_mode, drop_p, fmt, *wb):
+    def forward(ctx, x, ndir, hn_mode, drop_p, fmt, link, *wb):
         ctx.set_materialize_grads(False)
         _need_gpu(x, *wb)
         x = x.contiguous()
@@ -504,7 +523,11 @@
         b_ih = [wb[4 * d + 2].contiguous() for d in range(ndir)]
         b_hh = [wb[4 * d + 3].contiguous() for d in range(ndir)]
         H = w_hh[0].shape[1]
-        plan = ctx.plan = gru_layer_plan(T, B, In, H, ndir, drop_p, fmt)
+        site_in = link.site if link is not None else None
+        if site_in is not None and (x.data_ptr() != site_in.y_ptr or tuple(x.shape) != site_in.y_shape):
+            site_in = None
+        ctx.site_in = site_in
+        plan = ctx.plan = gru_layer_plan(T, B, In, H, ndir, drop_p, fmt, site_in, ctx.needs_input_grad[0])
         gi = torch.empty(ndir, T, B, 3 * H, dtype=_f32, device=x.device)
         if plan.w_fmt:
             w_ih = [split4(w) for w in w_ih]
@@ -538,6 +561,9 @@
             else:
                 call('xps_dropout_f32', _ptr(y), _ptr(out), None, out.numel(), drop[0], drop[1], _stream())
             y = out
+        ctx.site_out = None
+        if link is not None:
+            link.site = ctx.site_out = DropSite(drop[0], drop[1], plan.drop_fused, y) if drop is not None else None
         if hn_mode == HN_NONE:
             hn = None
         elif hn_mode == HN_SUM:
@@ -562,7 +588,16 @@
         w_ih, w_hh = w[:ndir], w[ndir:]
         fmt, y_fmt, x_fmt, w_fmt = plan.bwd_split4, plan.y_fmt, plan.x_fmt, plan.w_fmt
         wb = ctx.params
-        if ctx.drop is not None and dy is not None and not plan.drop_fused:
+        site_out = ctx.site_out
+        masked = False
+        if site_out is not None and site_out.applied:
+            held, site_out.dx, site_out.applied = site_out.dx, None, False
+            if dy is None or dy.data_ptr() != held.data_ptr() or dy.shape != held.shape:
+                raise RuntimeError('GRU backward: the next layer masked its input gradient for this layer (DropLink), but the '
+                                   'gradient that arrives here is not that tensor: a linked dropped output must reach the '
+                                   'next layer only')
+            masked = True
+        if ctx.drop is not None and dy is not None and not plan.drop_fused and not masked:
             dyc = dy.contiguous()
             dyd = torch.empty_like(dyc)
             call('xps_dropout_f32', _ptr(dyc), _ptr(dyd), None, dyc.numel(), ctx.drop[0], ctx.drop[1], _stream())
@@ -594,7 +629,14 @@
                 w_fmt, ldw = 1, 256
             else:
                 ldw = In
-            if ndir == 2:
+            if plan.dx_drop:
+                site = ctx.site_in
+                ra, rb, rc = rowmap(3 * H, fmt=fmt), rowmap(ldw, fmt=w_fmt), rowmap(In)
+                call('xps_gemm_nn2_drop_f32', _ptr(dgi[0]), _ptr(w_ih[0]), 3 * H, _ptr(dgi[1]) if ndir == 2 else None,
+                     _ptr(w_ih[1]) if ndir == 2 else None, 3 * H, C.byref(ra), C.byref(rb), _ptr(dx), C.byref(rc), T * B, In, 0,
+                     site.p, site.seed, _stream())
+                site.dx, site.applied = dx, True
+            elif ndir == 2:
                 ra, rb, rc = rowmap(3 * H, fmt=fmt), rowmap(ldw, fmt=w_fmt), rowmap(In)
                 call('xps_gemm_nn2_f32', _ptr(dgi[0]), _ptr(w_ih[0]), 3 * H, _ptr(dgi[1]), _ptr(w_ih[1]), 3 * H,
                      C.byref(ra), C.byref(rb), _ptr(dx), C.byref(rc), T * B, In, 0, _stream())
@@ -603,19 +645,19 @@
         grads = []
         for d in range(ndir):
             grads += [rets_ih[d][0], rets_hh[d][0], rets_ih[d][1], rets_hh[d][1]]
-        return (dx, None, None, None, None, *grads)
+        return (dx, None, None, None, None, None, *grads)
 
 
 class GRULayerDropFn(torch.autograd.Function):
 
     @staticmethod
     def forward(ctx, x, ndir, hn_mode, drop_p, *wb):
-        return GRULayerFmtFn.forward(ctx, x, ndir, hn_mode, drop_p, 0, *wb)
+        return GRULayerFmtFn.forward(ctx, x, ndir, hn_mode, drop_p, 0, None, *wb)
 
     @staticmethod
     def backward(ctx, dy, dhn):
         g = GRULayerFmtFn.backward(ctx, dy, dhn)
-        return g[:4] + g[5:]
+        return g[:4] + g[6:]
 
 
 class GRULayerFn(torch.autograd.Function):
diff --git a/cross_patient_speech_decoding_amd/nn_models/models.py b/cross_patient_speech_decoding_amd/nn_models/models.py
--- a/cross_patient_speech_decoding_amd/nn_models/models.py
+++ b/cross_patient_speech_decoding_amd/nn_models/models.py
@@ -126,12 +126,13 @@
         L = rnn.num_layers
         y = x
         fmt = 0
+        link = XF.DropLink()
         for l in range(L):
             p_drop = float(rnn.dropout) if (l < L - 1 and self.training) else 0.0
             T_, B_ = y.shape[0], y.shape[1]
             out_split = XF.layer_output_split4_ok(T_, B_, rnn.hidden_size, 2, p_drop)
             y, last = XF.GRULayerFmtFn.apply(y, 2, XF.HN_SUM if l == L - 1 else XF.HN_NONE, p_drop,
-                                             fmt | (XF.FMT_Y_SPLIT4 if out_split else 0), *_gru_layer_weights(rnn, l, 2))
+                                             fmt | (XF.FMT_Y_SPLIT4 if out_split else 0), link, *_gru_layer_weights(rnn, l, 2))
             fmt = XF.FMT_X_SPLIT4 if out_split else 0
         return y, last
 
@@ -326,9 +327,10 @@
         rnn = self.gru
         L = rnn.num_layers
         y, hn = z, None
+        link = XF.DropLink()
         for l in range(L):
             p_drop = float(rnn.dropout) if (l < L - 1 and self.training) else 0.0
-            y, hn = XF.GRULayerFmtFn.apply(y, 1, XF.HN_SUM if l == L - 1 else XF.HN_NONE, p_drop, 0,
+            y, hn = XF.GRULayerFmtFn.apply(y, 1, XF.HN_SUM if l == L - 1 else XF.HN_NONE, p_drop, 0, link,
                                            *_gru_layer_weights(rnn, l, 1))
         return XF.linear(hn, self.fc.weight, self.fc.bias)
 
diff --git a/include/xps.h b/include/xps.h
--- a/include/xps.h
+++ b/include/xps.h
@@ -44,6 +44,9 @@
 int xps_gemm_nn2_f32(const float* A1, const float* B1, int K1, const float* A2, const float* B2, int K2,
                      const xps_rowmap* ra, const xps_rowmap* rb, float* C, const xps_rowmap* rc,
                      int M, int N, int accumulate, void* stream);
+int xps_gemm_nn2_drop_f32(const float* A1, const float* B1, int K1, const float* A2, const float* B2, int K2,
+                          const xps_rowmap* ra, const xps_rowmap* rb, float* C, const xps_rowmap* rc,
+                          int M, int N, int accumulate, float drop_p, uint64_t drop_seed, void* stream);
 size_t xps_gemm_tn_f32_workspace(int M, int N, int K);
 int xps_gemm_tn_f32(const float* A, const xps_rowmap* ra, const float* B, const xps_rowmap* rb,
                     float* C, const xps_rowmap* rc,
```

Result: slower. 323,400 trials/s (-1.5%).
